# t-taniai/LocalExpStereo

Measured on AMD Instinct MI355X. Metric: Mcost-evals/s (pixels x hypotheses / s), guided-filter cost aggregation, 1500x1000x256 vol, higher is better.
Workload: dtype i32 fixed-point box sums (exact; i64 stage-2 window sums), f32 3x3 algebra and combination

## Files before the change

localexpstereo_amd/csrc/les_hip.hip:

```cpp
#include "../../include/localexp_hip.h"
#include "les_kernels.h"
#include "les_march.h"
#include "les_propose.h"
#include "les_post.h"
#include "les_pairwise.h"
#include "les_maxflow.h"
#include "les_maxflow_tiled.h"
#include "les_maxflow_cell.h"

#include "../host/ResidualCut.h"

#include <algorithm>
#include <atomic>
#include <chrono>
#include <cstdint>
#include <mutex>
#if !defined(LES_SIM)
#include <dlfcn.h>
#endif
#include <cstdarg>
#include <cstdio>
#include <cstdlib>
#include <cstring>
#include <string>
#include <vector>

namespace {

thread_local std::string g_err;

int fail(int code, const char* fmt, ...)
{
    char buf[512];
    va_list ap;
    va_start(ap, fmt);
    vsnprintf(buf, sizeof buf, fmt, ap);
    va_end(ap);
    g_err = buf;
    return code;
}

enum FallbackReason { FB_RADIUS = 0, FB_NONFINITE, FB_RANGE, FB_THRESHOLD, FB_IMAGE_SIZE, FB_GEOMETRY, FB_PATCHES, FB_GUIDE, FB_COUNT };
void note_fallback(std::atomic<unsigned>& seen, FallbackReason r, const char* fmt, ...)
{
    if (seen.fetch_or(1u << r, std::memory_order_relaxed) & (1u << r)) return;
    static const bool quiet = [] { const char* e = getenv("LES_HIP_QUIET"); return e && atoi(e) != 0; }();
    if (quiet) return;
    char buf[512];
    va_list ap;
    va_start(ap, fmt);
    vsnprintf(buf, sizeof buf, fmt, ap);
    va_end(ap);
    fprintf(stderr, "localexp_hip: strip kernel instead of the march kernel: %s (LES_HIP_QUIET=1 silences this note)\n", buf);
}

#define HIPCHECK(expr)                                                                               \
    do {                                                                                             \
        hipError_t e_ = (expr);                                                                      \
        if (e_ != hipSuccess)                                                                        \
            return fail(LES_HIP_ERR_DEVICE, "%s failed: %s (%s:%d)", #expr, hipGetErrorString(e_), __FILE__, __LINE__); \
    } while (0)

#include "les_hip_march_tables.inc"

struct ViewData {
    float* vol = nullptr;
    bool own_vol = false;
    float4* stats = nullptr;
    uint32_t* ipk = nullptr;
    uint32_t* ipk10 = nullptr;
    float4* feat = nullptr;
    uint32_t* ipk8 = nullptr;
    float* mstats = nullptr;
    float* vol_t = nullptr;
    bool march_ok = false;
    unsigned dmax_bits = 0;
    les::MarchView mv = {};
};

}

struct MtHost;
namespace { void mt_host_free(MtHost* m); }

struct les_hip_ctx {
    les_hip_params p;
    int R;
    const StripEntry* strip;
    const MarchEntry* march = nullptr;
    int ncu = 256;
    std::atomic<unsigned> fallback_seen{0};
    hipStream_t stream;
    les::Geom geom;
    ViewData v[2];
    float naive_alpha = 0;
    int naive = 0;
    float th_color = 0, th_grad = 0;
    float4* d_planes = nullptr; size_t planes_cap = 0;
    float* d_map = nullptr;
    les::WtaJob* d_wta = nullptr; size_t wta_cap = 0;
    float4* d_wta_planes = nullptr; size_t wta_planes_cap = 0;
    float* d_pw_tab = nullptr; float pw_omega = -1.f, pw_epsilon = -1.f;
    std::mutex mu;
    unsigned long long gen = 0;
    std::vector<les_hip_scratch*> idle_scratch;
    bool maxflow_lds_ready = false;
    bool maxflow_tiled_lds_ready = false;
    std::vector<les_hip_scratch*> own_scratch;
    std::vector<MtHost*> mt_idle;
};

struct les_hip_batch {
    int n = 0, njobs = 0, out_slabs = 0, R = 0;
    les::Job* d_jobs = nullptr;
    les::Job* d_mjobs = nullptr;
    const MarchEntry* mentry = nullptr;
    int nmgroups = 0;
    bool march_ok = false;
    les::RawCall* d_rawcalls = nullptr;
    long long* d_raw_off = nullptr;
    long long raw_floats = 0;
    int raw_chunks = 1;
    mutable float* d_raw[2] = {nullptr, nullptr};
    std::vector<les_hip_rect> targets;
    int device = 0;
    les::Rect4* d_units = nullptr;
    les::WtaJob* d_targets = nullptr;
    les::RansacScratch rs = {nullptr, nullptr, nullptr, nullptr, nullptr, nullptr, 0, nullptr};
    int wta_chunks = 1;
    int graph_chunks = 1;
    std::vector<long long> graph_off;
    long long graph_nodes = 0;
    long long* d_graph_off = nullptr;
    double* d_flow0 = nullptr;
    mutable std::mutex mt_mu;
    mutable les::MtTile* d_mt_tiles = nullptr;
    mutable int* d_mt_tiles_per_cell = nullptr;
    mutable int mt_ntiles = -1;
    mutable std::mutex mf_mu;
    mutable int* d_mf_list = nullptr;
    mutable int mf_list_key = -1;
    mutable int mf_count[3] = {0, 0, 0};
};

struct les_hip_scratch {
    les_hip_ctx* c = nullptr;
    hipStream_t stream = nullptr;
    float* d_tile = nullptr; float* h_tile = nullptr; size_t tile_cap = 0;
    float4* d_plane = nullptr; float4* h_plane = nullptr;
    struct Entry { les_hip_rect f, t; int want_march; const void* march; int njobs, ngroups; les::Job* d_jobs; unsigned long long stamp; };
    float* d_raw = nullptr; size_t raw_cap = 0;
    les::RawCall* d_rawcall = nullptr; long long* d_raw_off = nullptr;
    les_hip_rect raw_f = {-1, -1, -1, -1};
    std::vector<Entry> cache;
    unsigned long long clock = 0;
};

namespace {

std::atomic<unsigned long long> g_ctx_gen{0};
std::mutex g_live_mu;
std::vector<std::pair<unsigned long long, les_hip_ctx*>> g_live;
void release_hidden_scratch(unsigned long long gen, les_hip_scratch* s)
{
    std::lock_guard<std::mutex> lk(g_live_mu);
    for (auto& e : g_live)
        if (e.first == gen) {
            std::lock_guard<std::mutex> lk2(e.second->mu);
            e.second->idle_scratch.push_back(s);
            return;
        }
}
thread_local unsigned long long tl_stream_gen = 0;
thread_local hipStream_t tl_stream = nullptr;
inline hipStream_t cur_stream(const les_hip_ctx* c) { return (tl_stream_gen != 0 && tl_stream_gen == c->gen) ? tl_stream : c->stream; }

#include "les_hip_march.inc"

float naive_alpha(const les_hip_ctx* c) { return c->naive_alpha; }

}

#include "les_hip_context.inc"
#include "les_hip_batch.inc"
#include "les_hip_cuts.inc"
#include "les_hip_ingest_post.inc"
#include "les_hip_exchange.inc"
```

localexpstereo_amd/csrc/les_hip_batch.inc:

```
extern "C" {

int les_hip_batch_create(les_hip_ctx* c, int n, const les_hip_rect* frs, const les_hip_rect* trs, int out_slabs, les_hip_batch** out)
{
    if (!c || !out || n < 0 || (n > 0 && (!frs || !trs))) return fail(LES_HIP_ERR_ARG, "null argument");
    if (out_slabs < 0) return fail(LES_HIP_ERR_ARG, "out_slabs must be 0 (one map) or the number of consecutive calls that share a slab");
    if (out_slabs > 1 && n % out_slabs != 0) return fail(LES_HIP_ERR_ARG, "out_slabs = %d does not divide the %d calls of the batch (slab i / out_slabs holds out_slabs consecutive calls; pass 1 for one slab per call)", out_slabs, n);
    *out = nullptr;
    std::vector<les::Job> jobs;
    int rc = build_jobs(c, n, frs, trs, out_slabs, jobs);
    if (rc) return rc;
    les_hip_batch* b = new les_hip_batch();
    b->n = n; b->njobs = (int)jobs.size(); b->out_slabs = out_slabs; b->R = c->R; b->device = c->p.device;
    b->targets.assign(trs, trs + n);
    {
        int max_area = 1;
        for (int i = 0; i < n; i++) max_area = std::max(max_area, trs[i].w * trs[i].h);
        b->wta_chunks = std::min(32, std::max(1, (max_area + 4095) / 4096));
        b->graph_chunks = std::min(256, std::max(1, (max_area + 255) / 256));
    }
    b->graph_off.resize((size_t)n);
    for (int i = 0; i < n; i++) {
        b->graph_off[i] = b->graph_nodes;
        b->graph_nodes += (long long)std::max(0, trs[i].w) * std::max(0, trs[i].h);
    }
    if (n > 0) {
        static_assert(sizeof(les::WtaJob) == sizeof(les_hip_rect), "rect layout");
        static_assert(sizeof(les::GraphCell) == sizeof(les_hip_rect), "rect layout");
        if (hipMalloc((void**)&b->d_graph_off, (size_t)n * sizeof(long long)) != hipSuccess ||
            hipMemcpy(b->d_graph_off, b->graph_off.data(), (size_t)n * sizeof(long long), hipMemcpyHostToDevice) != hipSuccess ||
            hipMalloc((void**)&b->d_flow0, (size_t)n * b->graph_chunks * sizeof(double)) != hipSuccess) {
            les_hip_batch_destroy(b);
            return fail(LES_HIP_ERR_DEVICE, "upload of the graph offset table failed");
        }
        if (hipMalloc((void**)&b->d_targets, (size_t)n * sizeof(les::WtaJob)) != hipSuccess ||
            hipMemcpy(b->d_targets, trs, (size_t)n * sizeof(les::WtaJob), hipMemcpyHostToDevice) != hipSuccess) {
            les_hip_batch_destroy(b);
            return fail(LES_HIP_ERR_DEVICE, "upload of the target table failed");
        }
    }
    {
        std::vector<les::Job> mjobs;
        bool mok = false;
        build_march_jobs(c, n, frs, trs, out_slabs, mjobs, mok, b->mentry);
        if (mok && !mjobs.empty()) {
            if (hipMalloc((void**)&b->d_mjobs, mjobs.size() * sizeof(les::Job)) != hipSuccess ||
                hipMemcpy(b->d_mjobs, mjobs.data(), mjobs.size() * sizeof(les::Job), hipMemcpyHostToDevice) != hipSuccess) {
                les_hip_batch_destroy(b);
                return fail(LES_HIP_ERR_DEVICE, "upload of the march job table failed");
            }
            b->nmgroups = (int)(mjobs.size() / b->mentry->NJ);
            b->march_ok = true;
        }
        if (b->march_ok && c->naive) {
            std::vector<les::RawCall> calls((size_t)n);
            std::vector<long long> offs((size_t)n);
            long long tot = 0, amax = 1;
            for (int i = 0; i < n; i++) {
                const bool live = trs[i].w > 0 && trs[i].h > 0;
                const long long a = live ? (long long)frs[i].w * frs[i].h : 0;
                calls[i] = les::RawCall{frs[i].x, frs[i].y, live ? frs[i].w : 0, live ? frs[i].h : 0, tot};
                offs[i] = tot;
                tot += a; amax = std::max(amax, a);
            }
            if (tot > kRawPatchCapFloats) {
                b->march_ok = false;
                note_fallback(c->fallback_seen, FB_PATCHES, "the raw-cost patches of one batch of the image-based energy exceed 4 GB");
            }
            else {
                b->raw_floats = tot;
                b->raw_chunks = (int)std::min<long long>(1024, std::max<long long>(1, (amax + 4095) / 4096));
                if (hipMalloc((void**)&b->d_rawcalls, (size_t)n * sizeof(les::RawCall)) != hipSuccess ||
                    hipMemcpy(b->d_rawcalls, calls.data(), (size_t)n * sizeof(les::RawCall), hipMemcpyHostToDevice) != hipSuccess ||
                    hipMalloc((void**)&b->d_raw_off, (size_t)n * sizeof(long long)) != hipSuccess ||
                    hipMemcpy(b->d_raw_off, offs.data(), (size_t)n * sizeof(long long), hipMemcpyHostToDevice) != hipSuccess) {
                    les_hip_batch_destroy(b);
                    return fail(LES_HIP_ERR_DEVICE, "upload of the raw-cost call table failed");
                }
            }
        }
    }
    if (!jobs.empty()) {
        if (hipMalloc((void**)&b->d_jobs, jobs.size() * sizeof(les::Job)) != hipSuccess) { les_hip_batch_destroy(b); return fail(LES_HIP_ERR_DEVICE, "hipMalloc(jobs) failed"); }
        if (hipMemcpy(b->d_jobs, jobs.data(), jobs.size() * sizeof(les::Job), hipMemcpyHostToDevice) != hipSuccess) {
            les_hip_batch_destroy(b); return fail(LES_HIP_ERR_DEVICE, "hipMemcpy(jobs) failed");
        }
    }
    *out = b;
    return LES_HIP_OK;
}

void les_hip_batch_destroy(les_hip_batch* b)
{
    if (!b) return;
    if (b->d_jobs) (void)hipFree(b->d_jobs);
    if (b->d_mjobs) (void)hipFree(b->d_mjobs);
    if (b->d_rawcalls) (void)hipFree(b->d_rawcalls);
    if (b->d_raw_off) (void)hipFree(b->d_raw_off);
    for (int m = 0; m < 2; m++) if (b->d_raw[m]) (void)hipFree(b->d_raw[m]);
    if (b->d_units) (void)hipFree(b->d_units);
    if (b->d_targets) (void)hipFree(b->d_targets);
    if (b->d_graph_off) (void)hipFree(b->d_graph_off);
    if (b->d_flow0) (void)hipFree(b->d_flow0);
    if (b->d_mt_tiles) (void)hipFree(b->d_mt_tiles);
    if (b->d_mt_tiles_per_cell) (void)hipFree(b->d_mt_tiles_per_cell);
    if (b->d_mf_list) (void)hipFree(b->d_mf_list);
    if (b->rs.disp) (void)hipFree(b->rs.disp);
    if (b->rs.idx) (void)hipFree(b->rs.idx);
    if (b->rs.state) (void)hipFree(b->rs.state);
    if (b->rs.noi) (void)hipFree(b->rs.noi);
    if (b->rs.no) (void)hipFree(b->rs.no);
    if (b->rs.refit) (void)hipFree(b->rs.refit);
    if (b->rs.cell) (void)hipFree(b->rs.cell);
    delete b;
}

int les_hip_batch_set_units(les_hip_ctx* c, les_hip_batch* b, const les_hip_rect* units)
{
    if (!c || !b || (b->n > 0 && !units)) return fail(LES_HIP_ERR_ARG, "null argument");
    int maxlen = 1;
    for (int i = 0; i < b->n; i++) {
        const les_hip_rect& u = units[i];
        if (u.w <= 0 || u.h <= 0 || u.x < 0 || u.y < 0 || u.x + u.w > c->p.W || u.y + u.h > c->p.H)
            return fail(LES_HIP_ERR_ARG, "unit rect %d empty or outside the image", i);
        maxlen = std::max(maxlen, u.w * u.h);
    }
    if (b->n == 0) return LES_HIP_OK;
    static_assert(sizeof(les::Rect4) == sizeof(les_hip_rect), "rect layout");
    if (!b->d_units) HIPCHECK(hipMalloc((void**)&b->d_units, (size_t)b->n * sizeof(les::Rect4)));
    HIPCHECK(hipMemcpy(b->d_units, units, (size_t)b->n * sizeof(les::Rect4), hipMemcpyHostToDevice));
    if (!b->rs.idx) {
        const size_t n = (size_t)b->n, S = kRansacMaxSam;
        HIPCHECK(hipMalloc((void**)&b->rs.idx, n * S * 3 * sizeof(int)));
        HIPCHECK(hipMalloc((void**)&b->rs.state, n * (S + 1) * sizeof(uint64_t)));
        HIPCHECK(hipMalloc((void**)&b->rs.noi, n * S * sizeof(int)));
        HIPCHECK(hipMalloc((void**)&b->rs.no, n * S * sizeof(int)));
        HIPCHECK(hipMalloc((void**)&b->rs.refit, n * S * 3 * sizeof(float)));
        HIPCHECK(hipMalloc((void**)&b->rs.cell, n * sizeof(les::RansacCell)));
    }
    if (b->rs.disp) HIPCHECK(hipFree(b->rs.disp));
    b->rs.disp = nullptr;
    b->rs.stride = maxlen;
    HIPCHECK(hipMalloc((void**)&b->rs.disp, (size_t)b->n * maxlen * sizeof(float)));
    return LES_HIP_OK;
}

int les_hip_batch_propose(les_hip_ctx* c, const les_hip_batch* b, int kind, int m, les_hip_plane* labels, uint64_t* rng,
                          les_hip_plane* planes)
{
    if (c) (void)hipSetDevice(c->p.device);
    if (!c || !b || !labels || !rng || !planes) return fail(LES_HIP_ERR_ARG, "null argument");
    if (b->n == 0) return LES_HIP_OK;
    if (!b->d_units) return fail(LES_HIP_ERR_ARG, "les_hip_batch_set_units was not called for this batch");
    float4* lab = reinterpret_cast<float4*>(labels);
    float4* pl = reinterpret_cast<float4*>(planes);
    const int n = b->n, W = c->p.W;
    const float mind = c->p.min_disparity, maxd = c->p.max_disparity;
    switch (kind) {
    case LES_HIP_PROPOSE_EXPANSION:
        hipLaunchKernelGGL(les::les_expansion_kernel, dim3((n + 63) / 64), dim3(64), 0, cur_stream(c), b->d_units, lab, W, rng, pl, n);
        break;
    case LES_HIP_PROPOSE_RANDOM:
        hipLaunchKernelGGL(les::les_random_kernel, dim3((n + 63) / 64), dim3(64), 0, cur_stream(c), b->d_units, lab, W, rng, pl, n, m, mind, maxd);
        break;
    case LES_HIP_PROPOSE_RANSAC:
        hipLaunchKernelGGL(les::les_ransac_snapshot_kernel, dim3(n), dim3(256), 0, cur_stream(c), b->d_units, lab, W, b->rs);
        hipLaunchKernelGGL(les::les_ransac_begin_kernel, dim3((n + 63) / 64), dim3(64), 0, cur_stream(c), b->d_units, rng, b->rs, n, kRansacMaxSam, kRansacChunkEnds[0]);
        for (int k = 0, j0 = 0; k < kRansacChunks; k++) {
            const int j1 = kRansacChunkEnds[k], j2 = k + 1 < kRansacChunks ? kRansacChunkEnds[k + 1] : kRansacMaxSam;
            hipLaunchKernelGGL(les::les_ransac_eval_kernel, dim3(n, (j1 - j0 + les::kRansacCandPerBlock - 1) / les::kRansacCandPerBlock), dim3(64 * les::kRansacCandPerBlock), 0, cur_stream(c), b->d_units, b->rs, kRansacMaxSam, 1.0f, j0, j1);
            hipLaunchKernelGGL(les::les_ransac_walk_kernel, dim3((n + 63) / 64), dim3(64), 0, cur_stream(c), b->d_units, rng, pl, b->rs, n, kRansacMaxSam, 0.95f, j0, j1, j2);
            j0 = j1;
        }
        break;
    case LES_HIP_PROPOSE_INIT:
        hipLaunchKernelGGL(les::les_init_labels_kernel, dim3(n), dim3(64), 0, cur_stream(c), b->d_units, lab, W, rng, pl, mind, maxd);
        break;
    default:
        return fail(LES_HIP_ERR_ARG, "unknown proposer kind %d", kind);
    }
    HIPCHECK(hipGetLastError());
    return LES_HIP_OK;
}

int les_hip_batch_wta(les_hip_ctx* c, const les_hip_batch* b, const les_hip_plane* planes, float* cur, const float* prop,
                      les_hip_plane* labels)
{
    if (c) (void)hipSetDevice(c->p.device);
    if (!c || !b || !planes || !cur || !prop || !labels) return fail(LES_HIP_ERR_ARG, "null argument");
    if (b->n == 0) return LES_HIP_OK;
    if (!b->d_targets) return fail(LES_HIP_ERR_ARG, "batch has no target table");
    hipLaunchKernelGGL(les::les_wta_kernel, dim3(b->n, b->wta_chunks), dim3(256), 0, cur_stream(c), b->d_targets, reinterpret_cast<const float4*>(planes),
                       cur, prop, reinterpret_cast<float4*>(labels), c->p.W);
    HIPCHECK(hipGetLastError());
    return LES_HIP_OK;
}

int les_hip_batch_num_jobs(const les_hip_batch* b) { return b ? (b->march_ok ? b->nmgroups : b->njobs) : 0; }

int les_hip_batch_kernel_kind(const les_hip_ctx* c, const les_hip_batch* b, int mode)
{
    if (!c || !b || mode < 0 || mode > 1) return -1;
    return (b->march_ok && c->march && c->v[mode].march_ok) ? 1 : 0;
}

int les_hip_batch_run(les_hip_ctx* c, const les_hip_batch* b, int mode, const les_hip_plane* planes, int planes_on_device,
                      float* out_dev, int check)
{
    if (c) (void)hipSetDevice(c->p.device);
    if (!c || !b || !out_dev || (b->n > 0 && !planes)) return fail(LES_HIP_ERR_ARG, "null argument");
    if (b->R != c->R) return fail(LES_HIP_ERR_ARG, "batch was prepared for a different context");
    const float4* d_planes = reinterpret_cast<const float4*>(planes);
    if (!planes_on_device) {
        int rc = ensure_planes(c, (size_t)b->n);
        if (rc) return rc;
        HIPCHECK(hipMemcpyAsync(c->d_planes, planes, (size_t)b->n * sizeof(float4), hipMemcpyHostToDevice, cur_stream(c)));
        d_planes = c->d_planes;
    }
    if (b->march_ok && mode >= 0 && mode <= 1 && c->march && c->v[mode].march_ok) {
        if (!c->naive) return launch_march(c, b->mentry, mode, b->d_mjobs, b->nmgroups, d_planes, out_dev, check, cur_stream(c));
        {
            std::lock_guard<std::mutex> lk(c->mu);
            if (!b->d_raw[mode]) HIPCHECK(hipMalloc((void**)&b->d_raw[mode], (size_t)std::max<long long>(b->raw_floats, 1) * sizeof(float)));
        }
        const RawPatches rp{b->d_rawcalls, b->d_raw_off, b->d_raw[mode], b->n, b->raw_chunks};
        return launch_march(c, b->mentry, mode, b->d_mjobs, b->nmgroups, d_planes, out_dev, check, cur_stream(c), &rp);
    }
    return launch_strips(c, mode, b->d_jobs, b->njobs, d_planes, out_dev, check, cur_stream(c));
}

int les_hip_unary_batch(les_hip_ctx* c, int mode, int n, const les_hip_rect* frs, const les_hip_rect* trs,
                        const les_hip_plane* planes, float* cost_map, int check)
{
    if (!c || !cost_map) return fail(LES_HIP_ERR_ARG, "null argument");
    les_hip_batch* b = nullptr;
    int rc = les_hip_batch_create(c, n, frs, trs, 0, &b);
    if (rc) return rc;
    rc = les_hip_batch_run(c, b, mode, planes, 0, c->d_map, check);
    if (rc == LES_HIP_OK) {
        for (int i = 0; i < n && rc == LES_HIP_OK; i++) {
            const les_hip_rect& t = trs[i];
            if (t.w <= 0 || t.h <= 0) continue;
            size_t off = (size_t)t.y * c->p.W + t.x;
            hipError_t e = hipMemcpy2DAsync(cost_map + off, (size_t)c->p.W * sizeof(float), c->d_map + off, (size_t)c->p.W * sizeof(float),
                                            (size_t)t.w * sizeof(float), (size_t)t.h, hipMemcpyDeviceToHost, cur_stream(c));
            if (e != hipSuccess) rc = fail(LES_HIP_ERR_DEVICE, "hipMemcpy2DAsync failed: %s", hipGetErrorString(e));
        }
        if (rc == LES_HIP_OK && hipStreamSynchronize(cur_stream(c)) != hipSuccess) rc = fail(LES_HIP_ERR_DEVICE, "stream synchronize failed");
    }
    les_hip_batch_destroy(b);
    return rc;
}

int les_hip_scratch_create(les_hip_ctx* c, les_hip_scratch** out)
{
    if (!c || !out) return fail(LES_HIP_ERR_ARG, "null argument");
    *out = nullptr;
    HIPCHECK(hipSetDevice(c->p.device));
    les_hip_scratch* s = new les_hip_scratch();
    s->c = c;
    if (hipStreamCreateWithFlags(&s->stream, hipStreamNonBlocking) != hipSuccess ||
        hipMalloc((void**)&s->d_plane, sizeof(float4)) != hipSuccess || hipHostMalloc((void**)&s->h_plane, sizeof(float4), hipHostMallocDefault) != hipSuccess) {
        les_hip_scratch_destroy(s);
        return fail(LES_HIP_ERR_DEVICE, "scratch allocation failed");
    }
    *out = s;
    return LES_HIP_OK;
}

void les_hip_scratch_destroy(les_hip_scratch* s)
{
    if (!s) return;
    if (s->c) (void)hipSetDevice(s->c->p.device);
    if (s->stream) { (void)hipStreamSynchronize(s->stream); (void)hipStreamDestroy(s->stream); }
    for (auto& e : s->cache) if (e.d_jobs) (void)hipFree(e.d_jobs);
    if (s->d_tile) (void)hipFree(s->d_tile);
    if (s->h_tile) (void)hipHostFree(s->h_tile);
    if (s->d_raw) (void)hipFree(s->d_raw);
    if (s->d_rawcall) (void)hipFree(s->d_rawcall);
    if (s->d_raw_off) (void)hipFree(s->d_raw_off);
    if (s->d_plane) (void)hipFree(s->d_plane);
    if (s->h_plane) (void)hipHostFree(s->h_plane);
    delete s;
}

int les_hip_unary_one_scratch(les_hip_ctx* c, les_hip_scratch* s, int mode, const les_hip_rect* fr, const les_hip_rect* tr,
                              const les_hip_plane* plane, float* costs, int row_stride, int check)
{
    if (!c || !s || !fr || !tr || !plane || !costs) return fail(LES_HIP_ERR_ARG, "null argument");
    if (s->c != c) return fail(LES_HIP_ERR_ARG, "scratch belongs to another context");
    if (mode < 0 || mode > 1 || !c->v[mode].stats || (c->naive ? !c->v[1 - mode].feat : !c->v[mode].vol))
        return fail(LES_HIP_ERR_ARG, "view %d was not supplied at creation", mode);
    HIPCHECK(hipSetDevice(c->p.device));
    int rc = check_rects(c, *fr, *tr);
    if (rc) return rc;
    if (tr->w <= 0 || tr->h <= 0) return LES_HIP_OK;
    const int want_march = (c->march && c->v[mode].march_ok) ? 1 : 0;
    les_hip_scratch::Entry* e = nullptr;
    for (auto& x : s->cache)
        if (x.want_march == want_march && !memcmp(&x.f, fr, sizeof *fr) && !memcmp(&x.t, tr, sizeof *tr)) { e = &x; break; }
    if (!e) {
        std::vector<les::Job> jobs;
        bool mok = false;
        const MarchEntry* me = nullptr;
        if (want_march) build_march_jobs(c, 1, fr, tr, 0, jobs, mok, me);
        const bool use_march = want_march && mok && !jobs.empty();
        if (!use_march) {
            rc = build_jobs(c, 1, fr, tr, 0, jobs);
            if (rc) return rc;
            me = nullptr;
        }
        for (auto& j : jobs) {
            j.out_off = (long long)(j.ty0 - tr->y) * tr->w + (j.tx0 - tr->x);
            j.out_stride = tr->w;
        }
        les_hip_scratch::Entry ne{*fr, *tr, want_march, me, (int)jobs.size(), me ? (int)(jobs.size() / me->NJ) : 0, nullptr, 0};
        if (s->cache.size() >= 16) {
            size_t k = 0;
            for (size_t i = 1; i < s->cache.size(); i++) if (s->cache[i].stamp < s->cache[k].stamp) k = i;
            HIPCHECK(hipStreamSynchronize(s->stream));
            if (s->cache[k].d_jobs) HIPCHECK(hipFree(s->cache[k].d_jobs));
            s->cache.erase(s->cache.begin() + (long)k);
        }
        HIPCHECK(hipMalloc((void**)&ne.d_jobs, jobs.size() * sizeof(les::Job)));
        if (hipMemcpy(ne.d_jobs, jobs.data(), jobs.size() * sizeof(les::Job), hipMemcpyHostToDevice) != hipSuccess) {
            (void)hipFree(ne.d_jobs);
            return fail(LES_HIP_ERR_DEVICE, "upload of the job table failed");
        }
        s->cache.push_back(ne);
        e = &s->cache.back();
    }
    e->stamp = ++s->clock;
    const size_t need = (size_t)tr->w * tr->h;
    if (need > s->tile_cap) {
        HIPCHECK(hipStreamSynchronize(s->stream));
        if (s->d_tile) HIPCHECK(hipFree(s->d_tile));
        if (s->h_tile) HIPCHECK(hipHostFree(s->h_tile));
        s->d_tile = nullptr; s->h_tile = nullptr; s->tile_cap = 0;
        const size_t cap = std::max(need, (size_t)256 * 256);
        HIPCHECK(hipMalloc((void**)&s->d_tile, cap * sizeof(float)));
        HIPCHECK(hipHostMalloc((void**)&s->h_tile, cap * sizeof(float), hipHostMallocDefault));
        s->tile_cap = cap;
    }
    *s->h_plane = make_float4(plane->a, plane->b, plane->c, plane->v);
    HIPCHECK(hipMemcpyAsync(s->d_plane, s->h_plane, sizeof(float4), hipMemcpyHostToDevice, s->stream));
    if (e->march && c->naive) {
        const size_t rneed = (size_t)fr->w * fr->h;
        if (rneed > s->raw_cap || !s->d_rawcall) {
            HIPCHECK(hipStreamSynchronize(s->stream));
            if (s->d_raw) HIPCHECK(hipFree(s->d_raw));
            s->d_raw = nullptr; s->raw_cap = 0;
            const size_t cap = std::max(rneed, (size_t)256 * 256);
            HIPCHECK(hipMalloc((void**)&s->d_raw, cap * sizeof(float)));
            s->raw_cap = cap;
            if (!s->d_rawcall) {
                HIPCHECK(hipMalloc((void**)&s->d_rawcall, sizeof(les::RawCall)));
                HIPCHECK(hipMalloc((void**)&s->d_raw_off, sizeof(long long)));
                const long long zero = 0;
                HIPCHECK(hipMemcpy(s->d_raw_off, &zero, sizeof zero, hipMemcpyHostToDevice));
            }
            s->raw_f = les_hip_rect{-1, -1, -1, -1};
        }
        if (memcmp(&s->raw_f, fr, sizeof *fr)) {
            const les::RawCall call{fr->x, fr->y, fr->w, fr->h, 0};
            HIPCHECK(hipStreamSynchronize(s->stream));
            HIPCHECK(hipMemcpy(s->d_rawcall, &call, sizeof call, hipMemcpyHostToDevice));
            s->raw_f = *fr;
        }
        const RawPatches rp{s->d_rawcall, s->d_raw_off, s->d_raw, 1, (int)std::min<size_t>(1024, (rneed + 4095) / 4096)};
        rc = launch_march(c, static_cast<const MarchEntry*>(e->march), mode, e->d_jobs, e->ngroups, s->d_plane, s->d_tile, check, s->stream, &rp);
    }
    else if (e->march) rc = launch_march(c, static_cast<const MarchEntry*>(e->march), mode, e->d_jobs, e->ngroups, s->d_plane, s->d_tile, check, s->stream);
    else rc = launch_strips(c, mode, e->d_jobs, e->njobs, s->d_plane, s->d_tile, check, s->stream);
    if (rc) return rc;
    HIPCHECK(hipMemcpyAsync(s->h_tile, s->d_tile, need * sizeof(float), hipMemcpyDeviceToHost, s->stream));
    HIPCHECK(hipStreamSynchronize(s->stream));
    float* dst = costs + (size_t)(tr->y - fr->y) * row_stride + (tr->x - fr->x);
    for (int y = 0; y < tr->h; y++) memcpy(dst + (size_t)y * row_stride, s->h_tile + (size_t)y * tr->w, (size_t)tr->w * sizeof(float));
    return LES_HIP_OK;
}

int les_hip_unary_one(les_hip_ctx* c, int mode, const les_hip_rect* fr, const les_hip_rect* tr, const les_hip_plane* plane,
                      float* costs, int row_stride, int check)
{
    if (!c || !fr || !tr || !plane || !costs) return fail(LES_HIP_ERR_ARG, "null argument");
    struct Mine {
        std::vector<std::pair<unsigned long long, les_hip_scratch*>> v;
        ~Mine() { for (auto& e : v) release_hidden_scratch(e.first, e.second); }
    };
    thread_local Mine mine;
    les_hip_scratch* s = nullptr;
    for (auto& e : mine.v) if (e.first == c->gen) { s = e.second; break; }
    if (!s) {
        {
            std::lock_guard<std::mutex> lk(c->mu);
            if (!c->idle_scratch.empty()) { s = c->idle_scratch.back(); c->idle_scratch.pop_back(); }
        }
        if (!s) {
            int rc = les_hip_scratch_create(c, &s);
            if (rc) return rc;
            std::lock_guard<std::mutex> lk(c->mu);
            c->own_scratch.push_back(s);
        }
        mine.v.emplace_back(c->gen, s);
    }
    return les_hip_unary_one_scratch(c, s, mode, fr, tr, plane, costs, row_stride, check);
}

int les_hip_wta_update(les_hip_ctx* c, int n, const les_hip_rect* rects, const les_hip_plane* planes, int planes_on_device,
                       float* cur, const float* prop, les_hip_plane* labels)
{
    if (!c || n < 0 || (n > 0 && (!rects || !planes || !cur || !prop || !labels))) return fail(LES_HIP_ERR_ARG, "null argument");
    if (n == 0) return LES_HIP_OK;
    for (int i = 0; i < n; i++)
        if (rects[i].x < 0 || rects[i].y < 0 || rects[i].w < 0 || rects[i].h < 0 || rects[i].x + rects[i].w > c->p.W || rects[i].y + rects[i].h > c->p.H)
            return fail(LES_HIP_ERR_ARG, "rect outside the image");
    if ((size_t)n > c->wta_cap) {
        if (c->d_wta) HIPCHECK(hipFree(c->d_wta));
        c->d_wta = nullptr; c->wta_cap = 0;
        HIPCHECK(hipMalloc((void**)&c->d_wta, std::max<size_t>(n, 1024) * sizeof(les::WtaJob)));
        c->wta_cap = std::max<size_t>(n, 1024);
    }
    static_assert(sizeof(les::WtaJob) == sizeof(les_hip_rect), "rect layout");
    HIPCHECK(hipMemcpyAsync(c->d_wta, rects, (size_t)n * sizeof(les::WtaJob), hipMemcpyHostToDevice, cur_stream(c)));
    const float4* d_planes = reinterpret_cast<const float4*>(planes);
    if (!planes_on_device) {
        if ((size_t)n > c->wta_planes_cap) {
            if (c->d_wta_planes) HIPCHECK(hipFree(c->d_wta_planes));
            c->d_wta_planes = nullptr; c->wta_planes_cap = 0;
            HIPCHECK(hipMalloc((void**)&c->d_wta_planes, std::max<size_t>(n, 1024) * sizeof(float4)));
            c->wta_planes_cap = std::max<size_t>(n, 1024);
        }
        HIPCHECK(hipMemcpyAsync(c->d_wta_planes, planes, (size_t)n * sizeof(float4), hipMemcpyHostToDevice, cur_stream(c)));
        d_planes = c->d_wta_planes;
    }
    int max_area = 1;
    for (int i = 0; i < n; i++) max_area = std::max(max_area, rects[i].w * rects[i].h);
    const int chunks = std::min(32, std::max(1, (max_area + 4095) / 4096));
    hipLaunchKernelGGL(les::les_wta_kernel, dim3(n, chunks), dim3(256), 0, cur_stream(c), c->d_wta, d_planes, cur, prop,
                       reinterpret_cast<float4*>(labels), c->p.W);
    HIPCHECK(hipGetLastError());
    return LES_HIP_OK;
}

}
```

localexpstereo_amd/csrc/les_hip_context.inc:

```
extern "C" {

const char* les_hip_last_error(void) { return g_err.c_str(); }

#if defined(LES_PHASE_TIMING)
int les_hip_debug_phases(unsigned long long* out)
{
    (void)hipDeviceSynchronize();
    if (hipMemcpyFromSymbol(out, HIP_SYMBOL(les::les_dbg), 12 * sizeof(unsigned long long)) != hipSuccess) return 1;
    unsigned long long z[12] = {0, 0, 0, 0, 0, 0, 0, 0, 0, 0, 0, 0};
    (void)hipMemcpyToSymbol(HIP_SYMBOL(les::les_dbg), z, sizeof z);
    return 0;
}
#endif

int les_hip_strip_width(int R)
{
    const StripEntry* e = find_strip(R);
    return e ? e->TW : 0;
}

static int create_common(les_hip_ctx** out, const les_hip_params* params, const uint8_t* imL, const uint8_t* imR,
                         const float* volL, const float* volR, int naive, float alpha, float th_grad)
{
    if (!out || !params) return fail(LES_HIP_ERR_ARG, "null argument");
    *out = nullptr;
    les_hip_params p = *params;
    if (naive) { p.D = 1; p.volumes_on_device = 0; }
    if (p.H <= 0 || p.W <= 0 || p.D <= 0 || p.windR < 2) return fail(LES_HIP_ERR_ARG, "bad dimensions");
    if (naive && (!imL || !imR)) return fail(LES_HIP_ERR_ARG, "the image-based matching cost needs both views");
    if ((unsigned long long)p.H * p.W * p.D >= (1ull << 32)) return fail(LES_HIP_ERR_UNSUPPORTED, "volumes of 2^32 or more floats are not supported (32-bit element offsets)");
    const StripEntry* strip = naive ? find_naive_strip(p.windR / 2) : find_strip(p.windR / 2);
    if (!strip) return fail(LES_HIP_ERR_UNSUPPORTED, "no kernel instantiated for guided-filter radius %d (windR %d)", p.windR / 2, p.windR);
    int ndev = 0;
    if (hipGetDeviceCount(&ndev) != hipSuccess || ndev <= 0) return fail(LES_HIP_ERR_DEVICE, "no HIP device available (this library has no CPU fallback)");
    if (p.device < 0 || p.device >= ndev) return fail(LES_HIP_ERR_ARG, "device %d out of range (%d devices)", p.device, ndev);
    HIPCHECK(hipSetDevice(p.device));
    les_hip_ctx* c = new les_hip_ctx();
    c->gen = ++g_ctx_gen;
    { std::lock_guard<std::mutex> lk(g_live_mu); g_live.emplace_back(c->gen, c); }
    c->p = p;
    c->R = p.windR / 2;
    c->strip = strip;
    c->march = find_march(p.windR / 2);
    if (!c->march && !(getenv("LES_HIP_KERNEL") && !strcmp(getenv("LES_HIP_KERNEL"), "strip")))
        note_fallback(c->fallback_seen, FB_RADIUS, "no march kernel for guided-filter radius %d (windR %d; instantiated: 2 .. 10)", p.windR / 2, p.windR);
#if !defined(LES_SIM)
    {
        int v = 0;
        if (hipDeviceGetAttribute(&v, hipDeviceAttributeMultiprocessorCount, p.device) == hipSuccess && v > 0) c->ncu = v;
    }
#endif
    c->stream = nullptr;
    c->geom.H = p.H; c->geom.W = p.W; c->geom.D = p.D;
    c->geom.D0 = (int)(-p.min_disparity);
    c->geom.th_col = p.th_col; c->geom.pad_ = 0.0f;
    c->geom.maxd = p.max_disparity; c->geom.mind = p.min_disparity;
    c->naive = naive;
    if (naive) {
        c->th_color = p.th_col * (1.0f - alpha);
        c->th_grad = th_grad * alpha;
        c->naive_alpha = alpha;
    }
    const uint8_t* ims[2] = {imL, imR};
    const float* vols[2] = {volL, volR};
    for (int m = 0; m < 2; m++) {
        int rc = build_view(c, m, ims[m], vols[m]);
        if (rc) { les_hip_destroy(c); return rc; }
    }
    if (hipMalloc((void**)&c->d_map, (size_t)p.H * p.W * sizeof(float)) != hipSuccess) {
        les_hip_destroy(c);
        return fail(LES_HIP_ERR_DEVICE, "hipMalloc of the scratch cost map failed");
    }
    *out = c;
    return LES_HIP_OK;
}

int les_hip_create(les_hip_ctx** out, const les_hip_params* params, const uint8_t* imL, const uint8_t* imR,
                   const float* volL, const float* volR)
{
    return create_common(out, params, imL, imR, volL, volR, 0, 0.0f, 0.0f);
}

int les_hip_create_naive(les_hip_ctx** out, const les_hip_params* params, const uint8_t* imL, const uint8_t* imR, float alpha, float th_grad)
{
    return create_common(out, params, imL, imR, nullptr, nullptr, 1, alpha, th_grad);
}

void les_hip_destroy(les_hip_ctx* c)
{
    if (!c) return;
    (void)hipSetDevice(c->p.device);
    if (tl_stream_gen == c->gen) { tl_stream_gen = 0; tl_stream = nullptr; }
    {
        std::lock_guard<std::mutex> lk(g_live_mu);
        g_live.erase(std::remove_if(g_live.begin(), g_live.end(), [c](const std::pair<unsigned long long, les_hip_ctx*>& e) { return e.second == c; }), g_live.end());
    }
    for (int m = 0; m < 2; m++) {
        if (c->v[m].own_vol && c->v[m].vol) (void)hipFree(c->v[m].vol);
        if (c->v[m].stats) (void)hipFree(c->v[m].stats);
        if (c->v[m].ipk) (void)hipFree(c->v[m].ipk);
        if (c->v[m].ipk10) (void)hipFree(c->v[m].ipk10);
        if (c->v[m].feat) (void)hipFree(c->v[m].feat);
        if (c->v[m].ipk8) (void)hipFree(c->v[m].ipk8);
        if (c->v[m].mstats) (void)hipFree(c->v[m].mstats);
        if (c->v[m].vol_t) (void)hipFree(c->v[m].vol_t);
    }
    for (les_hip_scratch* sc : c->own_scratch) les_hip_scratch_destroy(sc);
    c->own_scratch.clear();
    for (MtHost* m : c->mt_idle) mt_host_free(m);
    c->mt_idle.clear();
    if (c->d_planes) (void)hipFree(c->d_planes);
    if (c->d_map) (void)hipFree(c->d_map);
    if (c->d_wta) (void)hipFree(c->d_wta);
    if (c->d_wta_planes) (void)hipFree(c->d_wta_planes);
    if (c->d_pw_tab) (void)hipFree(c->d_pw_tab);
    delete c;
}

int les_hip_set_stream(les_hip_ctx* c, void* s)
{
    if (!c) return fail(LES_HIP_ERR_ARG, "null context");
    c->stream = (hipStream_t)s;
    return LES_HIP_OK;
}

int les_hip_set_thread_stream(les_hip_ctx* c, void* s, int bind)
{
    if (!c) return fail(LES_HIP_ERR_ARG, "null context");
    if (bind) { tl_stream_gen = c->gen; tl_stream = (hipStream_t)s; }
    else if (tl_stream_gen == c->gen) { tl_stream_gen = 0; tl_stream = nullptr; }
    return LES_HIP_OK;
}

int les_hip_synchronize(les_hip_ctx* c)
{
    if (!c) return fail(LES_HIP_ERR_ARG, "null context");
    HIPCHECK(hipStreamSynchronize(cur_stream(c)));
    return LES_HIP_OK;
}

int les_hip_refresh_volume(les_hip_ctx* c, int mode)
{
    if (!c) return fail(LES_HIP_ERR_ARG, "null argument");
    if (mode < 0 || mode > 1 || !c->v[mode].vol) return fail(LES_HIP_ERR_ARG, "view %d has no cost volume", mode);
    HIPCHECK(hipSetDevice(c->p.device));
    std::lock_guard<std::mutex> lk(c->mu);
    HIPCHECK(hipStreamSynchronize(cur_stream(c)));
    if (!c->march || !c->v[mode].mstats) return LES_HIP_OK;
    const int rc = build_march_view(c, mode, nullptr);
    if (rc) return rc;
    HIPCHECK(hipStreamSynchronize(cur_stream(c)));
    return LES_HIP_OK;
}

int les_hip_calib_copy(const float* d_src, float* d_dst, size_t n, int device, void* stream)
{
    if (!d_src || !d_dst || n == 0) return fail(LES_HIP_ERR_ARG, "bad argument");
    HIPCHECK(hipSetDevice(device));
    hipLaunchKernelGGL(les::les_calib_copy_kernel, dim3((unsigned)((n + 255) / 256)), dim3(256), 0, (hipStream_t)stream, d_src, d_dst, n);
    HIPCHECK(hipGetLastError());
    return LES_HIP_OK;
}

int les_hip_calib_copy_wide(const float* d_src, float* d_dst, size_t n, int device, void* stream)
{
    if (!d_src || !d_dst || n == 0 || (n & 3) || (((uintptr_t)d_src | (uintptr_t)d_dst) & 15)) return fail(LES_HIP_ERR_ARG, "bad argument (n must be a multiple of 4, pointers 16-byte aligned)");
    HIPCHECK(hipSetDevice(device));
    const size_t n4 = n / 4;
    hipLaunchKernelGGL(les::les_calib_copy_wide_kernel, dim3((unsigned)((n4 + 1023) / 1024)), dim3(256), 0, (hipStream_t)stream,
                       reinterpret_cast<const float4*>(d_src), reinterpret_cast<float4*>(d_dst), n4);
    HIPCHECK(hipGetLastError());
    return LES_HIP_OK;
}

int les_hip_malloc(les_hip_ctx* c, void** p, size_t bytes)
{
    if (!c || !p) return fail(LES_HIP_ERR_ARG, "null argument");
    HIPCHECK(hipMalloc(p, bytes));
    return LES_HIP_OK;
}
int les_hip_free(les_hip_ctx* c, void* p)
{
    if (!c) return fail(LES_HIP_ERR_ARG, "null argument");
    if (p) HIPCHECK(hipFree(p));
    return LES_HIP_OK;
}
int les_hip_memcpy_h2d(les_hip_ctx* c, void* d, const void* s, size_t bytes)
{
    if (!c) return fail(LES_HIP_ERR_ARG, "null argument");
    HIPCHECK(hipMemcpyAsync(d, s, bytes, hipMemcpyHostToDevice, cur_stream(c)));
    HIPCHECK(hipStreamSynchronize(cur_stream(c)));
    return LES_HIP_OK;
}
int les_hip_memcpy_d2h(les_hip_ctx* c, void* d, const void* s, size_t bytes)
{
    if (!c) return fail(LES_HIP_ERR_ARG, "null argument");
    HIPCHECK(hipMemcpyAsync(d, s, bytes, hipMemcpyDeviceToHost, cur_stream(c)));
    HIPCHECK(hipStreamSynchronize(cur_stream(c)));
    return LES_HIP_OK;
}
int les_hip_memset(les_hip_ctx* c, void* d, int value, size_t bytes)
{
    if (!c) return fail(LES_HIP_ERR_ARG, "null argument");
    HIPCHECK(hipMemsetAsync(d, value, bytes, cur_stream(c)));
    return LES_HIP_OK;
}

size_t les_hip_tiled_volume_bytes(les_hip_ctx* c, int mode)
{
    if (!c || mode < 0 || mode > 1 || !c->v[mode].vol_t) return 0;
    return (size_t)c->p.H * (size_t)((c->p.W + 7) / 8) * 8u * (size_t)c->p.D * sizeof(float);
}

int les_hip_get_stats(les_hip_ctx* c, int mode, float* out)
{
    if (!c || !out || mode < 0 || mode > 1 || !c->v[mode].stats) return fail(LES_HIP_ERR_ARG, "bad argument");
    HIPCHECK(hipMemcpy(out, c->v[mode].stats, (size_t)c->p.H * c->p.W * 12 * sizeof(float), hipMemcpyDeviceToHost));
    return LES_HIP_OK;
}

}
```

localexpstereo_amd/csrc/les_hip_march.inc:

```
int check_rects(const les_hip_ctx* c, const les_hip_rect& f, const les_hip_rect& t)
{
    if (f.w < 0 || f.h < 0 || t.w < 0 || t.h < 0) return fail(LES_HIP_ERR_ARG, "negative rect size");
    if (f.x < 0 || f.y < 0 || f.x + f.w > c->p.W || f.y + f.h > c->p.H) return fail(LES_HIP_ERR_ARG, "filterRect outside the image");
    if (t.w > 0 && t.h > 0 && (t.x < f.x || t.y < f.y || t.x + t.w > f.x + f.w || t.y + t.h > f.y + f.h))
        return fail(LES_HIP_ERR_ARG, "targetRect not inside filterRect");
    return LES_HIP_OK;
}

int build_jobs(const les_hip_ctx* c, int n, const les_hip_rect* frs, const les_hip_rect* trs, int out_slabs,
               std::vector<les::Job>& jobs)
{
    const int TW = c->strip->TW, R = c->R;
    const long long P = (long long)c->p.H * c->p.W;
    long long strips = 0;
    for (int i = 0; i < n; i++) {
        int rc = check_rects(c, frs[i], trs[i]);
        if (rc) return rc;
        if (trs[i].w > 0 && trs[i].h > 0) strips += (trs[i].w + TW - 1) / TW;
    }
    int max_rows = 1 << 30;
    if (strips > 0 && strips < 2048) {
        long long want = (2048 + strips - 1) / strips;
        int tallest = 0;
        for (int i = 0; i < n; i++) tallest = std::max(tallest, trs[i].h);
        max_rows = std::max<long long>(std::max(8 * R, 64), (tallest + want - 1) / want);
    }
    jobs.clear();
    for (int i = 0; i < n; i++) {
        const les_hip_rect &f = frs[i], &t = trs[i];
        if (t.w <= 0 || t.h <= 0) continue;
        for (int sy = 0; sy < t.h; sy += max_rows)
            for (int sx = 0; sx < t.w; sx += TW) {
                les::Job j;
                j.tx0 = t.x + sx; j.ty0 = t.y + sy;
                j.tw = std::min(TW, t.w - sx); j.th = std::min(max_rows, t.h - sy);
                j.cx0 = f.x; j.cy0 = f.y; j.cx1 = f.x + f.w; j.cy1 = f.y + f.h;
                j.out_off = (out_slabs ? (long long)(i / out_slabs) * P : 0) + (long long)j.ty0 * c->p.W + j.tx0;
                j.out_stride = c->p.W;
                j.plane_idx = i;
                jobs.push_back(j);
            }
    }
    std::stable_sort(jobs.begin(), jobs.end(), [](const les::Job& a, const les::Job& b) {
        if (a.tx0 != b.tx0) return a.tx0 < b.tx0;
        if (a.ty0 != b.ty0) return a.ty0 < b.ty0;
        return a.plane_idx < b.plane_idx;
    });
    return LES_HIP_OK;
}

bool build_march_jobs(les_hip_ctx* c, int n, const les_hip_rect* frs, const les_hip_rect* trs, int out_slabs,
                      std::vector<les::Job>& jobs, bool& ok, const MarchEntry*& entry)
{
    jobs.clear();
    ok = false;
    entry = nullptr;
    if (!c->march) return true;
    const int R = c->R, W = c->p.W, H = c->p.H;
    const long long P = (long long)H * W;
    ok = true;
    for (int i = 0; i < n; i++) {
        const les_hip_rect &f = frs[i], &t = trs[i];
        if (t.w <= 0 || t.h <= 0) continue;
        if ((f.x > 0 && t.x - f.x < 2 * R) || (f.x + f.w < W && (f.x + f.w) - (t.x + t.w) < 2 * R) ||
            (f.y > 0 && t.y - f.y < 2 * R) || (f.y + f.h < H && (f.y + f.h) - (t.y + t.h) < 2 * R)) ok = false;
    }
    if (!ok) {
        note_fallback(c->fallback_seen, FB_GEOMETRY, "a target rectangle lies closer than 2 x radius = %d pixels to a filterRect border that is not an image border", 2 * R);
        return true;
    }
    const int ncu = c->ncu;
    const MarchEntry* cands[2] = {c->march, find_march(c->R, 0)};
    const MarchEntry* m = c->march;
    int max_rows = 1 << 30;
    {
        double best = 1e300;
        const int row_opts[] = {1 << 30, 1024, 512, 384, 256, 192, 128, 96, 64, 48, 32};
        for (int g = 0; g < 2; g++) {
            const MarchEntry* e = cands[g];
            if (!e || (g == 1 && e == cands[0])) continue;
            if (const char* w = getenv("LES_HIP_MARCH_WIDE")) if ((atoi(w) != 0) != (g == 0)) continue;
            for (int ro : row_opts) {
                long long njobs = 0;
                int rows = 0, useful = 0;
                for (int i = 0; i < n; i++) {
                    const les_hip_rect& t = trs[i];
                    if (t.w <= 0 || t.h <= 0) continue;
                    const int ns = (t.w + e->TW - 1) / e->TW;
                    const int nr = (t.h + ro - 1) / ro, sh = (t.h + nr - 1) / nr;
                    njobs += (long long)ns * nr;
                    rows = std::max(rows, sh);
                    useful = std::max(useful, (t.w + ns - 1) / ns);
                }
                if (njobs == 0) continue;
                const long long wgs = (njobs + e->NJ - 1) / e->NJ;
                const double ticks = (double)((rows + 4 * R + e->BY - 1) / e->BY + 3);
                const double cost = (double)((wgs + ncu - 1) / ncu) * ticks * (1.0 + 1e-3 * (double)wgs / ncu) + (ro == (1 << 30) ? 0.0 : 1e-6);
                if (cost < best) { best = cost; m = e; max_rows = ro; }
            }
        }
    }
    if (const char* e = getenv("LES_HIP_MARCH_ROWS")) max_rows = std::max(1, atoi(e));
    entry = m;
    const int TW = m->TW, NJ = m->NJ;
    for (int i = 0; i < n; i++) {
        const les_hip_rect &f = frs[i], &t = trs[i];
        if (t.w <= 0 || t.h <= 0) continue;
        const int ns = (t.w + TW - 1) / TW, sw = (t.w + ns - 1) / ns;
        const int nr = (t.h + max_rows - 1) / max_rows, sh = (t.h + nr - 1) / nr;
        for (int sy = 0; sy < t.h; sy += sh)
            for (int sx = 0; sx < t.w; sx += sw) {
                les::Job j;
                j.tx0 = t.x + sx; j.ty0 = t.y + sy;
                j.tw = std::min(sw, t.w - sx); j.th = std::min(sh, t.h - sy);
                j.cx0 = f.x; j.cy0 = f.y; j.cx1 = f.x + f.w; j.cy1 = f.y + f.h;
                j.out_off = (out_slabs ? (long long)(i / out_slabs) * P : 0) + (long long)j.ty0 * W + j.tx0;
                j.out_stride = W;
                j.plane_idx = i;
                jobs.push_back(j);
            }
    }
    std::stable_sort(jobs.begin(), jobs.end(), [](const les::Job& a, const les::Job& b) {
        if (a.tx0 != b.tx0) return a.tx0 < b.tx0;
        if (a.ty0 != b.ty0) return a.ty0 < b.ty0;
        return a.plane_idx < b.plane_idx;
    });
    while (!jobs.empty() && jobs.size() % NJ) {
        les::Job pad = jobs.back();
        pad.tw = 0; pad.th = 0;
        jobs.push_back(pad);
    }
    return true;
}

int ensure_planes(les_hip_ctx* c, size_t n)
{
    if (n <= c->planes_cap) return LES_HIP_OK;
    if (c->d_planes) HIPCHECK(hipFree(c->d_planes));
    c->d_planes = nullptr; c->planes_cap = 0;
    size_t cap = std::max<size_t>(n, 1024);
    HIPCHECK(hipMalloc((void**)&c->d_planes, cap * sizeof(float4)));
    c->planes_cap = cap;
    return LES_HIP_OK;
}

struct RawPatches { const les::RawCall* calls; const long long* off; float* raw; int n, chunks; };

les::View strip_view(const les_hip_ctx* c, int mode)
{
    les::View view{c->v[mode].vol, c->v[mode].stats, c->v[mode].ipk, c->v[mode].ipk10, nullptr, nullptr, mode ? -1.0f : 1.0f, c->th_color, c->th_grad};
    if (c->naive) { view.feat_self = c->v[mode].feat; view.feat_other = c->v[1 - mode].feat; }
    return view;
}

int launch_march(les_hip_ctx* c, const MarchEntry* m, int mode, const les::Job* d_mjobs, int ngroups, const float4* d_planes, float* d_out, int check,
                 hipStream_t stream, const RawPatches* rp = nullptr)
{
    if (ngroups <= 0) return LES_HIP_OK;
    les::MarchView mv = c->v[mode].mv;
    if (c->naive) {
        if (!rp || !rp->raw || !c->v[1 - mode].feat) return fail(LES_HIP_ERR_ARG, "view %d was not supplied at creation", mode);
        hipLaunchKernelGGL(les::les_naive_raw_kernel, dim3(rp->n, rp->chunks), dim3(256), 0, stream, c->geom, strip_view(c, mode), rp->calls, d_planes, rp->raw);
        mv.vol = rp->raw; mv.raw_off = rp->off;
    }
    hipLaunchKernelGGL(m->fn, dim3(ngroups), dim3(m->NT), 0, stream, c->geom, mv, d_mjobs, d_planes, d_out, ngroups, check);
    HIPCHECK(hipGetLastError());
    return LES_HIP_OK;
}

int launch_strips(les_hip_ctx* c, int mode, const les::Job* d_jobs, int njobs, const float4* d_planes, float* d_out, int check, hipStream_t stream)
{
    if (njobs <= 0) return LES_HIP_OK;
    if (mode < 0 || mode > 1 || !c->v[mode].stats || (c->naive ? !c->v[1 - mode].feat : !c->v[mode].vol))
        return fail(LES_HIP_ERR_ARG, "view %d was not supplied at creation", mode);
    const les::View view = strip_view(c, mode);
    hipLaunchKernelGGL(c->strip->fn, dim3(njobs), dim3(c->strip->NT), 0, stream, c->geom, view, d_jobs, d_planes, d_out, njobs, check);
    HIPCHECK(hipGetLastError());
    return LES_HIP_OK;
}

float naive_alpha(const les_hip_ctx* c);

int build_march_view(les_hip_ctx* c, int m, const double* d_hs)
{
    ViewData& v = c->v[m];
    const size_t P = (size_t)c->p.H * c->p.W;
    const int W = c->p.W, H = c->p.H;
    v.march_ok = false;
    if ((unsigned long long)P * (4ull * les::kMarchStatWords) >= (1ull << 31)) {
        note_fallback(c->fallback_seen, FB_IMAGE_SIZE, "image of %d x %d pixels (32-bit row offsets reach 2^26 pixels)", W, H);
        return LES_HIP_OK;
    }
    const float th = c->naive ? c->th_color + c->th_grad : c->p.th_col;
    if (!(th > 0.0f) || !(th < INFINITY)) { note_fallback(c->fallback_seen, FB_THRESHOLD, "truncation threshold %g is not positive and finite", (double)th); return LES_HIP_OK; }
    if (d_hs) {
        unsigned dbits = 0;
        struct DevBuf { void* p = nullptr; ~DevBuf() { if (p) (void)hipFree(p); } } dm;
        HIPCHECK(hipMalloc(&dm.p, sizeof(unsigned)));
        unsigned* d_dmax = static_cast<unsigned*>(dm.p);
        HIPCHECK(hipMemsetAsync(d_dmax, 0, sizeof(unsigned), cur_stream(c)));
        HIPCHECK(hipMalloc((void**)&v.ipk8, P * sizeof(uint32_t)));
        HIPCHECK(hipMalloc((void**)&v.mstats, P * les::kMarchStatWords * sizeof(float)));
        hipLaunchKernelGGL(les::les_march_stats_kernel, dim3((W + 255) / 256, H), dim3(256), 0, cur_stream(c), d_hs, v.ipk, v.ipk8, v.mstats, d_dmax, H, W, c->R, c->p.eps);
        HIPCHECK(hipGetLastError());
        HIPCHECK(hipMemcpyAsync(&dbits, d_dmax, sizeof(unsigned), hipMemcpyDeviceToHost, cur_stream(c)));
        HIPCHECK(hipStreamSynchronize(cur_stream(c)));
        v.dmax_bits = dbits;
    }
    auto drop_tiled = [&]() { if (v.vol_t) { (void)hipFree(v.vol_t); v.vol_t = nullptr; } };
    const int nb = 2048;
    std::vector<float> hmin(nb, 0.0f); std::vector<int> hbad(nb, 0);
    if (!c->naive) {
        struct DevBuf { void* p = nullptr; ~DevBuf() { if (p) (void)hipFree(p); } } part;
        HIPCHECK(hipMalloc(&part.p, nb * (sizeof(float) + sizeof(int))));
        float* d_min = static_cast<float*>(part.p);
        int* d_bad = reinterpret_cast<int*>(d_min + nb);
        hipLaunchKernelGGL(les::les_range_kernel, dim3(nb), dim3(256), 0, cur_stream(c), v.vol, P * (size_t)c->p.D, d_min, d_bad);
        HIPCHECK(hipGetLastError());
        HIPCHECK(hipMemcpyAsync(hmin.data(), d_min, nb * sizeof(float), hipMemcpyDeviceToHost, cur_stream(c)));
        HIPCHECK(hipMemcpyAsync(hbad.data(), d_bad, nb * sizeof(int), hipMemcpyDeviceToHost, cur_stream(c)));
        HIPCHECK(hipStreamSynchronize(cur_stream(c)));
    }
    float vmin = INFINITY; int bad = 0;
    for (int i = 0; i < nb; i++) { vmin = std::min(vmin, hmin[i]); bad |= hbad[i]; }
    if (bad || !(vmin < INFINITY)) {
        note_fallback(c->fallback_seen, FB_NONFINITE, "the cost volume of view %d holds NaN or infinite entries", m);
        drop_tiled();
        return LES_HIP_OK;
    }
    vmin = std::min(vmin, 0.5f * th);
    const double range = (double)th - (double)vmin;
    if (!(range <= 8.0 * (double)th)) {
        note_fallback(c->fallback_seen, FB_RANGE, "view %d: costs reach %g below the truncation threshold %g (more than 8 x the threshold)", m, range, (double)th);
        drop_tiled();
        return LES_HIP_OK;
    }
    const unsigned dbits = v.dmax_bits;
    float dmax;
    memcpy(&dmax, &dbits, sizeof dmax);
    if (!(dmax > 0.0f) || !(dmax < INFINITY)) { note_fallback(c->fallback_seen, FB_GUIDE, "view %d: the inverse covariance of the guide is not positive and finite (largest diagonal entry %g)", m, (double)dmax); return LES_HIP_OK; }
    const int K = 2 * c->R + 1;
    const double Ba = 0.5 * range * std::sqrt((double)dmax), Bb = range + 1.5 * Ba;
    const double scale = 1073741824.0 / ((double)K * Bb * 1.25);
    const int PB = les::march_pb(c->R);
    const float spf = (float)((double)((1 << PB) - 1) / range);
    const double c0 = std::rint(-(double)vmin * (double)spf) - (double)(1 << (PB - 1));
    const double up = 1.0 / (double)spf;
    les::MarchView mv;
    mv.vol = v.vol; mv.ipk8 = v.ipk8; mv.mstats = v.mstats;
    mv.sp = spf;
    mv.pmagic = (float)(12582912.0 + c0);
    mv.poff = (float)(-c0 * up);
    mv.kapS = (float)((double)(1 << les::kMarchSH) * up / 255.0 * scale);
    mv.upS = (float)(up * scale);
    mv.qscale = (float)((double)(1 << les::kMarchS2) / (255.0 * scale));
    mv.kmu = (float)(1.0 / ((double)(1ll << les::kMarchMB) * 255.0));
    mv.raw_off = nullptr;
    mv.vol_t = nullptr;
    if (!c->naive && v.vol) {
        const char* e = getenv("LES_HIP_TILED");
        const unsigned long long nt = (unsigned long long)H * (unsigned long long)((W + 7) / 8) * 8ull * (unsigned long long)c->p.D;
        if (!(e && atoi(e) == 0) && (unsigned long long)((W + 7) / 8) * (unsigned long long)c->p.D * 32ull < (1ull << 31)) {
            if (v.vol_t) { (void)hipFree(v.vol_t); v.vol_t = nullptr; }
            size_t mem_free = 0, mem_total = 0;
            const bool room = hipMemGetInfo(&mem_free, &mem_total) == hipSuccess && mem_free >= 2 * nt * sizeof(float) + (4ull << 30);
            if (room && hipMalloc((void**)&v.vol_t, nt * sizeof(float)) == hipSuccess) {
                hipLaunchKernelGGL(les::les_tile_volume_kernel, dim3((unsigned)(((W + 7) / 8 * 8 + 63) / 64), (unsigned)H), dim3(256), 0, cur_stream(c), v.vol, v.vol_t, c->p.D, H, W);
                HIPCHECK(hipGetLastError());
                mv.vol_t = v.vol_t;
            } else {
                (void)hipGetLastError();
                v.vol_t = nullptr;
            }
        }
    }
    v.mv = mv;
    v.march_ok = true;
    return LES_HIP_OK;
}

int build_view(les_hip_ctx* c, int m, const uint8_t* im, const float* vol)
{
    const size_t P = (size_t)c->p.H * c->p.W;
    ViewData& v = c->v[m];
    if (vol) {
        if (c->p.volumes_on_device) { v.vol = const_cast<float*>(vol); v.own_vol = false; }
        else {
            HIPCHECK(hipMalloc((void**)&v.vol, P * c->p.D * sizeof(float)));
            v.own_vol = true;
            HIPCHECK(hipMemcpy(v.vol, vol, P * c->p.D * sizeof(float), hipMemcpyHostToDevice));
        }
    }
    if (!im) return LES_HIP_OK;
    uint8_t* d_img = nullptr;
    double* d_hs = nullptr;
    HIPCHECK(hipMalloc((void**)&d_img, P * 3));
    HIPCHECK(hipMemcpy(d_img, im, P * 3, hipMemcpyHostToDevice));
    HIPCHECK(hipMalloc((void**)&v.ipk, P * sizeof(uint32_t)));
    HIPCHECK(hipMalloc((void**)&v.ipk10, P * sizeof(uint32_t)));
    HIPCHECK(hipMalloc((void**)&v.stats, (P * 3 + 1) * sizeof(float4)));
    HIPCHECK(hipMemsetAsync(v.stats + P * 3, 0, sizeof(float4), cur_stream(c)));
    HIPCHECK(hipMalloc((void**)&d_hs, P * 9 * sizeof(double)));
    const int W = c->p.W, H = c->p.H;
    if (c->naive) {
        HIPCHECK(hipMalloc((void**)&v.feat, P * sizeof(float4)));
        hipLaunchKernelGGL(les::les_naive_features_kernel, dim3((c->p.W + 255) / 256, c->p.H), dim3(256), 0, cur_stream(c), d_img, v.feat, c->p.H, c->p.W, naive_alpha(c));
    }
    hipLaunchKernelGGL(les::les_pack_guide_kernel, dim3((unsigned)((P + 255) / 256)), dim3(256), 0, cur_stream(c), d_img, v.ipk, v.ipk10, (int)P);
    hipLaunchKernelGGL(les::les_stats_hsum_kernel, dim3((W + 255) / 256, H), dim3(256), 0, cur_stream(c), v.ipk, d_hs, H, W, c->R);
    hipLaunchKernelGGL(les::les_stats_finish_kernel, dim3((W + 255) / 256, H), dim3(256), 0, cur_stream(c), d_hs, v.stats, H, W, c->R, c->p.eps);
    HIPCHECK(hipGetLastError());
    if (c->march && (v.vol || c->naive)) {
        int rc = build_march_view(c, m, d_hs);
        if (rc) { (void)hipFree(d_img); (void)hipFree(d_hs); return rc; }
    }
    HIPCHECK(hipStreamSynchronize(cur_stream(c)));
    HIPCHECK(hipFree(d_img));
    HIPCHECK(hipFree(d_hs));
    return LES_HIP_OK;
}
```

localexpstereo_amd/csrc/les_hip_march_tables.inc:

```
typedef void (*StripKernel)(les::Geom, les::View, const les::Job*, const float4*, float*, int, int);
struct StripEntry { int R; int variant; int TW; int NT; StripKernel fn; };

#define LES_STRIP_ENTRY(R_, V_, WA_, BY_, SEG_, MW_) \
    { R_, V_, les::StripCfg<R_, WA_, BY_, SEG_>::TW, les::StripCfg<R_, WA_, BY_, SEG_>::NT, les::les_strip_kernel<R_, WA_, BY_, SEG_, MW_> }
const StripEntry kStrips[] = {
    LES_STRIP_ENTRY(1, 0, 64, 16, 4, 2), LES_STRIP_ENTRY(2, 0, 64, 16, 4, 2), LES_STRIP_ENTRY(3, 0, 64, 16, 4, 2),
    LES_STRIP_ENTRY(4, 0, 64, 16, 4, 2), LES_STRIP_ENTRY(5, 0, 64, 16, 4, 2), LES_STRIP_ENTRY(6, 0, 64, 16, 4, 2),
    LES_STRIP_ENTRY(7, 0, 64, 16, 4, 2), LES_STRIP_ENTRY(8, 0, 64, 16, 4, 2), LES_STRIP_ENTRY(9, 0, 64, 16, 4, 2),
    LES_STRIP_ENTRY(10, 0, 64, 21, 3, 3), LES_STRIP_ENTRY(12, 0, 64, 16, 4, 2), LES_STRIP_ENTRY(15, 0, 96, 16, 6, 2),
    LES_STRIP_ENTRY(10, 8, 128, 21, 6, 2), LES_STRIP_ENTRY(10, 11, 64, 21, 3, 2),
};
#define LES_NAIVE_ENTRY(R_, WA_, BY_, SEG_, MW_) \
    { R_, 0, les::StripCfg<R_, WA_, BY_, SEG_>::TW, les::StripCfg<R_, WA_, BY_, SEG_>::NT, les::les_strip_kernel<R_, WA_, BY_, SEG_, MW_, 1> }
const StripEntry kNaiveStrips[] = {
    LES_NAIVE_ENTRY(1, 64, 16, 4, 2), LES_NAIVE_ENTRY(2, 64, 16, 4, 2), LES_NAIVE_ENTRY(3, 64, 16, 4, 2), LES_NAIVE_ENTRY(4, 64, 16, 4, 2),
    LES_NAIVE_ENTRY(5, 64, 16, 4, 2), LES_NAIVE_ENTRY(6, 64, 16, 4, 2), LES_NAIVE_ENTRY(7, 64, 16, 4, 2), LES_NAIVE_ENTRY(8, 64, 16, 4, 2),
    LES_NAIVE_ENTRY(9, 64, 16, 4, 2), LES_NAIVE_ENTRY(10, 64, 16, 4, 2), LES_NAIVE_ENTRY(12, 64, 16, 4, 2), LES_NAIVE_ENTRY(15, 96, 16, 6, 2),
};
const StripEntry* find_naive_strip(int R)
{
    for (const auto& e : kNaiveStrips)
        if (e.R == R) return &e;
    return nullptr;
}
const StripEntry* find_strip(int R)
{
    int variant = 0;
    if (const char* v = getenv("LES_HIP_VARIANT")) variant = atoi(v);
    const StripEntry* def = nullptr;
    for (const auto& e : kStrips) {
        if (e.R != R) continue;
        if (e.variant == variant) return &e;
        if (e.variant == 0) def = &e;
    }
    return def;
}

typedef void (*MarchKernel)(les::Geom, les::MarchView, const les::Job*, const float4*, float*, int, int);
struct MarchEntry { int R; int TW; int NJ; int NT; int BY; MarchKernel fn; };
#define LES_MARCH_ENTRY(R_, WGC_, NJ_, BY_) \
    { R_, les::MarchCfg<R_, WGC_, NJ_, BY_>::TW, NJ_, les::MarchCfg<R_, WGC_, NJ_, BY_>::NT, BY_, les::les_march_kernel<R_, WGC_, NJ_, BY_> }
const MarchEntry kMarch[] = {
    LES_MARCH_ENTRY(10, 256, 1, 7),
#if defined(LES_MARCH_LAB) && defined(LES_MARCH_NARROW_NJ1)
    LES_MARCH_ENTRY(10, 128, 1, 7),
#else
    LES_MARCH_ENTRY(10, 128, 2, 7),
#endif
    LES_MARCH_ENTRY(7, 256, 1, 5),
    LES_MARCH_ENTRY(7, 128, 2, 5),
#if !defined(LES_MARCH_FEW_RADII)
    LES_MARCH_ENTRY(2, 256, 1, 2),  LES_MARCH_ENTRY(2, 128, 2, 2),
    LES_MARCH_ENTRY(3, 256, 1, 3),  LES_MARCH_ENTRY(3, 128, 2, 3),
    LES_MARCH_ENTRY(4, 256, 1, 3),  LES_MARCH_ENTRY(4, 128, 2, 3),
    LES_MARCH_ENTRY(5, 256, 1, 4),  LES_MARCH_ENTRY(5, 128, 2, 4),
    LES_MARCH_ENTRY(6, 256, 1, 5),  LES_MARCH_ENTRY(6, 128, 2, 5),
    LES_MARCH_ENTRY(8, 256, 1, 6),  LES_MARCH_ENTRY(8, 128, 2, 6),
    LES_MARCH_ENTRY(9, 256, 1, 7),  LES_MARCH_ENTRY(9, 128, 2, 7),
#endif
};
const MarchEntry* find_march(int R, int wide = 1)
{
    if (const char* k = getenv("LES_HIP_KERNEL")) if (!strcmp(k, "strip")) return nullptr;
    const MarchEntry* best = nullptr;
    for (const auto& e : kMarch)
        if (e.R == R && (!best || (wide ? e.TW > best->TW : e.TW < best->TW))) best = &e;
    return best;
}

constexpr long long kRawPatchCapFloats = 1ll << 30;
constexpr int kRansacMaxSam = 500;
constexpr int kRansacChunks = 5;
constexpr int kRansacChunkEnds[kRansacChunks] = {16, 64, 128, 256, kRansacMaxSam};
```

localexpstereo_amd/csrc/les_kernels.h:

```cpp
#pragma once

#include "les_simt.h"

#include <utility>

namespace les {

struct Geom {
    int H, W, D, D0;
    float th_col, pad_;
    float maxd, mind;
};

struct View {
    const float* vol;
    const float4* stats;
    const uint32_t* ipk;
    const uint32_t* ipk10;
    const float4* feat_self;
    const float4* feat_other;
    float sign;
    float th_color, th_grad;
};

struct Job {
    int tx0, ty0, tw, th;
    int cx0, cy0, cx1, cy1;
    long long out_off;
    int out_stride;
    int plane_idx;
};

#define LES_COST_INVALID 1000000.0f

__device__ __forceinline__ float gather_cost(const Geom& g, const float* __restrict__ vol, float a, float b,
                                             float c, int gx, int gy)
{
    const size_t HW = (size_t)g.H * g.W;
    const size_t px = (size_t)gy * g.W + gx;
    float d_base = b * (float)gy + c;
    float d = a * (float)gx + d_base;
    float C;
    if (d < g.mind) C = vol[px];
    else if (d >= g.maxd) C = vol[(size_t)(g.D - 1) * HW + px];
    else if (d != d || fabsf(d) == INFINITY) C = LES_COST_INVALID;
    else {
        int d0 = (int)d + g.D0;
        int d1 = d0 + 1;
        float f1 = d - floorf(d);
        float f0 = 1.0f - f1;
        if (d1 >= g.D || d0 < 0) C = LES_COST_INVALID;
        else {
            float v0 = vol[(size_t)d0 * HW + px];
            float v1 = vol[(size_t)d1 * HW + px];
            C = f0 * v0 + f1 * v1;
        }
    }
    return (g.th_col < C) ? g.th_col : C;
}

struct GatherPrep {
    uint32_t i0, i1;
    float f1;
    int mode;
};
__device__ __forceinline__ GatherPrep gather_prepare(const Geom& g, float ax, float d_base, uint32_t px, uint32_t HW, bool inside)
{
    GatherPrep r;
    const float d = ax + d_base;
    const bool lo = d < g.mind, hi = d >= g.maxd;
    const bool mid = !(lo || hi || d != d);
    const float dsafe = mid ? d : 0.0f;
    const int d0 = (int)dsafe + g.D0;
    const bool ok = mid && d0 >= 0 && d0 + 1 < g.D;
    r.f1 = dsafe - floorf(dsafe);
    const uint32_t s0 = lo ? 0u : (hi ? (uint32_t)(g.D - 1) : (ok ? (uint32_t)d0 : 0u));
    r.i0 = s0 * HW + px;
    r.i1 = ok ? r.i0 + HW : r.i0;
    r.mode = !inside ? 3 : ((lo || hi) ? 1 : (ok ? 0 : 2));
    return r;
}
__device__ __forceinline__ float gather_finish(const Geom& g, const GatherPrep& r, float v0, float v1)
{
    const float f0 = 1.0f - r.f1;
    float C = f0 * v0 + r.f1 * v1;
    C = r.mode == 1 ? v0 : C;
    C = r.mode == 2 ? LES_COST_INVALID : C;
    const float p = (g.th_col < C) ? g.th_col : C;
    return r.mode == 3 ? 0.0f : p;
}

struct NaivePrep {
    uint32_t ia, ib;
    float w1;
};
__device__ __forceinline__ NaivePrep naive_prepare(const Geom& g, float sign, float a, float b, float c, int gx, int gy)
{
    NaivePrep r;
    const float z = (a * (float)gx + b * (float)gy) + c;
    const double sx = (double)gx - (double)sign * (double)z;
    const double q = floor(sx * 32.0 + 0.5) / 32.0;
    const double fl = floor(q);
    r.w1 = (float)(q - fl);
    const double flc = fmin(fmax(fl, -2.0), (double)g.W + 1.0);
    const int x0 = (int)flc;
    const int xa = min(max(x0, 0), g.W - 1), xb = min(max(x0 + 1, 0), g.W - 1);
    r.ia = (uint32_t)gy * (uint32_t)g.W + (uint32_t)xa;
    r.ib = (uint32_t)gy * (uint32_t)g.W + (uint32_t)xb;
    return r;
}
__device__ __forceinline__ float naive_finish(const View& v, const NaivePrep& r, float4 own, float4 fa, float4 fb)
{
    const float w0 = 1.0f - r.w1;
    const float v0 = w0 * fa.x + r.w1 * fb.x, v1 = w0 * fa.y + r.w1 * fb.y, v2 = w0 * fa.z + r.w1 * fb.z, v3 = w0 * fa.w + r.w1 * fb.w;
    const float col = (fabsf(own.x - v0) + fabsf(own.y - v1)) + fabsf(own.z - v2);
    const float grad = fabsf(own.w - v3);
    return ((col < v.th_color) ? col : v.th_color) + ((grad < v.th_grad) ? grad : v.th_grad);
}

__device__ __forceinline__ bool label_valid(const Geom& g, float a, float b, float c, float v, int gx, int gy)
{
    float fx = (float)gx, fy = (float)gy;
    float ds = ((fx * a + fy * b) + 1.0f * c) + 0.0f * v;
    float a5 = a * 5, b5 = b * 5;
    float d;
    return (ds >= g.mind && ds <= g.maxd
            && ((d = ds + a5 + b5) >= g.mind) && d <= g.maxd
            && ((d = ds + a5 - b5) >= g.mind) && d <= g.maxd
            && ((d = ds - a5 + b5) >= g.mind) && d <= g.maxd
            && ((d = ds - a5 - b5) >= g.mind) && d <= g.maxd);
}

__device__ __forceinline__ float guide_centred_f32(uint32_t ipk, int k)
{
    int u = (int)((ipk >> (8 * k)) & 0xffu);
    float w = (float)(2 * u - 255) * (1.0f / 510.0f);
    return k == 3 ? 1.0f : w;
}
__device__ __forceinline__ float guide10_field_f32(uint32_t w10, int off)
{
#if defined(LES_SIM)
    const int v = ((int)(w10 << (22 - off))) >> 22;
#else
    const int v = __builtin_amdgcn_sbfe((int)w10, (unsigned)off, 10u);
#endif
    return (float)v * (1.0f / 510.0f);
}
__device__ __forceinline__ float guide10_centred_f32(uint32_t w10, int k)
{
#if defined(LES_SIM)
    const int v = ((int)(w10 << (22 - 10 * (k < 3 ? k : 0)))) >> 22;
#else
    const int v = __builtin_amdgcn_sbfe((int)w10, (unsigned)(10 * k), 10u);
#endif
    const float w = (float)v * (1.0f / 510.0f);
    return k == 3 ? 1.0f : w;
}
__device__ __forceinline__ double guide_centred_f64(uint32_t ipk, int k)
{
    int u = (int)((ipk >> (8 * k)) & 0xffu);
    double w = fma((double)u, 1.0 / 255, -0.5);
    return k == 3 ? 1.0 : w;
}

__device__ __forceinline__ int window_count(int c, int R, int lo, int hi)
{
    int a = c - R < lo ? lo : c - R;
    int b = c + R + 1 > hi ? hi : c + R + 1;
    return b > a ? b - a : 0;
}

#if defined(LES_SIM)
#define LES_SCHED_FENCE(step) ((void)0)
#else
#define LES_SCHED_FENCE(step) do { if (((step) & 3) == 3) __builtin_amdgcn_sched_barrier(0); } while (0)
#endif
#if defined(LES_SIM)
#define LES_SCHED_FENCE_V(row) ((void)0)
#else
#define LES_SCHED_FENCE_V(row) do { if (((row) % 3) == 2) __builtin_amdgcn_sched_barrier(0); } while (0)
#endif

#ifndef LES_H1_F32
typedef double H1ACC;
#else
typedef float H1ACC;
#endif

template <int V>
struct IntTag { static constexpr int value = V; };

template <int... Is, typename F>
__device__ __forceinline__ void static_for_impl(std::integer_sequence<int, Is...>, F&& f)
{
    (f(IntTag<Is>{}), ...);
}
template <int N, typename F>
__device__ __forceinline__ void static_for(F&& f)
{
    static_for_impl(std::make_integer_sequence<int, N>{}, f);
}

template <int R, int RS>
struct VLane {
    static constexpr int KS = 2 * R + 1;
    static_assert(RS >= KS, "ring shorter than the window");
    float ring1[RS] = {};
    float ring2[RS] = {};
    double S1 = 0.0, S2 = 0.0;
    int k;

    template <int S>
    __device__ __forceinline__ float step(float in, bool keep, double rn1, float4 s)
    {
        constexpr int OLD = (S + RS - KS) % RS;
        S1 += (double)in - (double)ring1[OLD];
        ring1[S] = in;
        const double m = S1 * rn1;
        const double mp = quad_bcast<3>(m);
        const float cov = (float)fma(-(double)s.x, mp, m);
        const float ak = fmaf(s.w, quad_bcast<2>(cov), fmaf(s.z, quad_bcast<1>(cov), s.y * quad_bcast<0>(cov)));
        const float bb = (float)mp - quad_sum(ak * s.x);
        float val = (k < 3) ? ak : bb;
        if (!keep) val = 0.0f;
        S2 += (double)val - (double)ring2[OLD];
        ring2[S] = val;
        return (float)S2;
    }
};

template <int R, int WA, int BY, int SEG>
struct StripCfg {
    static constexpr int TW = WA - 2 * R;
    static constexpr int WP = WA + 2 * R;
    static constexpr int NT = 4 * WA;
    static constexpr int HL = 4 * BY * SEG;
    static constexpr int L1 = (WA + SEG - 1) / SEG;
    static constexpr int L2 = (TW + SEG - 1) / SEG;
    static constexpr int TPITCH = WA * 4 + 4;
    static constexpr int KS = 2 * R + 1;
    static constexpr int RS = ((KS + BY - 1) / BY) * BY;
    static_assert(HL <= NT, "more H lanes than threads");
    static_assert(TW > 0, "strip too narrow for this radius");
};

#if defined(LES_PHASE_TIMING) && !defined(LES_SIM)
__device__ unsigned long long les_dbg[12];
#define LES_PHASE_BEGIN() unsigned long long ph_[5] = {0, 0, 0, 0, 0}; unsigned long long tl_ = clock64()
#define LES_PHASE_MARK(k) do { const unsigned long long now_ = clock64(); ph_[k] += now_ - tl_; tl_ = now_; } while (0)
#define LES_PHASE_END() do { if (threadIdx.x == 0) { for (int k_ = 0; k_ < 5; k_++) atomicAdd(&les_dbg[k_], ph_[k_]); atomicAdd(&les_dbg[5], 1ull); } } while (0)
#else
#define LES_PHASE_BEGIN() ((void)0)
#define LES_PHASE_MARK(k) ((void)0)
#define LES_PHASE_END() ((void)0)
#endif

template <int R, int WA, int BY, int SEG, int MW, int SRC = 0>
__global__ void __launch_bounds__(4 * WA, MW)
les_strip_kernel(Geom g, View view, const Job* __restrict__ jobs, const float4* __restrict__ planes,
                 float* __restrict__ out, int njobs, int check)
{
    using Cfg = StripCfg<R, WA, BY, SEG>;
    constexpr int TW = Cfg::TW, WP = Cfg::WP, NT = Cfg::NT, HL = Cfg::HL, L1 = Cfg::L1, L2 = Cfg::L2;
    constexpr int TPITCH = Cfg::TPITCH, KS = Cfg::KS, RS = Cfg::RS;

    __shared__ float s_p[BY][WP];
    __shared__ uint32_t s_ipk[BY][WP];
    __shared__ float s_T[BY][TPITCH];
    __shared__ uint32_t s_ipk2[BY][TW];
    __shared__ double s_rtab[2 * R + 2];
    __shared__ uint32_t s_c510[WP];
    struct RowInfo { double rny; int flags; uint32_t soff; };
    __shared__ RowInfo s_row[BY];
    struct GRow { uint32_t rowpx; float d_base; };
    __shared__ GRow s_grow[BY];
    __shared__ double s_rnx2[TW + 4];
    __shared__ int s_gsy[BY];
    float (*s_q)[WP] = s_p;

    int job_id;
    {
        const int nwg = (int)gridDim.x, orig = (int)blockIdx.x;
        const int q = nwg / 8, r = nwg % 8, xcd = orig % 8;
        job_id = (xcd < r ? xcd * (q + 1) : r * (q + 1) + (xcd - r) * q) + orig / 8;
    }
    if (job_id >= njobs) return;
    const Job job = jobs[job_id];
    const float4 plane = planes[job.plane_idx];
    const int tid = (int)threadIdx.x;
    const int Ttot = job.th + 4 * R;

    if (tid < 2 * R + 2) s_rtab[tid] = tid > 0 ? 1.0 / (double)tid : 0.0;
    if (tid < WP) s_c510[tid] = 510u;

    const int vx = tid >> 2, vk = tid & 3;
    VLane<R, RS> vl;
    vl.k = vk;
    const int gx1 = job.tx0 - R + vx;
    const bool col_in_clip = gx1 >= job.cx0 && gx1 < job.cx1;
    const int nx1 = window_count(gx1, R, job.cx0, job.cx1);

    const bool h_active = tid < HL;
    const int hk = tid & 3, hrow = (tid >> 2) % BY, hseg = (tid >> 2) / BY;
    const uint32_t* h1_guide = hk < 3 ? &s_ipk[hrow][0] : &s_c510[0];
    const int h1_off = hk < 3 ? 10 * hk : 0;

    __syncthreads();
    const double rnx1 = s_rtab[nx1];

    constexpr int GRP = NT / WP, GPASS = (BY + GRP - 1) / GRP;
    constexpr int ORP = NT / TW, OPASS = (BY + ORP - 1) / ORP;
    const int g_ri = tid / WP, g_xi = tid - g_ri * WP;
    const bool g_lane = tid < GRP * WP;
    const int g_gx = job.tx0 - 2 * R + g_xi;
    const bool g_col_in = g_gx >= job.cx0 && g_gx < job.cx1;
    const int g_sx = min(max(g_gx, job.cx0), job.cx1 - 1);
    const float g_ax = plane.x * (float)g_sx;
    const int o_ri = tid / TW, o_xo = tid - o_ri * TW;
    const bool o_lane = tid < ORP * TW;
    const int o_sx = min(max(job.tx0 + o_xo, job.cx0), job.cx1 - 1);
    const uint32_t HWu = (uint32_t)g.H * (uint32_t)g.W;

    constexpr int PD = (BY % 4 == 0) ? 4 : ((BY % 3 == 0) ? 3 : 1);
    const int sgx1 = min(max(gx1, job.cx0), job.cx1 - 1);
    const float4* st_col = vk < 3 ? view.stats + (size_t)sgx1 * 3 + vk : view.stats + (size_t)g.H * g.W * 3;
    const size_t st_stride = (size_t)g.W * 3;
    auto stats_row = [&](int t) -> float4 {
        const int gy1 = min(max(job.ty0 - 3 * R + t, job.cy0), job.cy1 - 1);
        return st_col[(vk < 3 ? (size_t)gy1 : (size_t)0) * st_stride];
    };
    float4 pre[PD];
#pragma unroll
    for (int j = 0; j < PD; j++) pre[j] = stats_row(j);

    auto fill_row_tables = [&](int tb) {
        const int t = tb + tid;
        const int gy1 = job.ty0 - 3 * R + t;
        RowInfo ri;
        ri.rny = s_rtab[window_count(gy1, R, job.cy0, job.cy1)];
        ri.flags = ((gy1 >= job.cy0 && gy1 < job.cy1) ? 1 : 0) | (t >= 2 * R ? 2 : 0);
        ri.soff = (uint32_t)min(max(gy1 + PD, job.cy0), job.cy1 - 1) * (uint32_t)(g.W * 3);
        s_row[tid] = ri;
        const int gy = job.ty0 - 2 * R + t;
        GRow gr;
        const int sy = min(max(gy, job.cy0), job.cy1 - 1);
        gr.rowpx = ((uint32_t)sy * (uint32_t)g.W) | ((t < Ttot && gy >= job.cy0 && gy < job.cy1) ? 0x80000000u : 0u);
        gr.d_base = plane.y * (float)sy + plane.z;
        s_grow[tid] = gr;
        if constexpr (SRC == 1) s_gsy[tid] = sy;
    };
    if (tid < BY) fill_row_tables(0);
    if (tid < TW + 4) s_rnx2[tid] = s_rtab[window_count(job.tx0 + tid, R, job.cx0, job.cx1)];
    __syncthreads();

    LES_PHASE_BEGIN();
    for (int t0 = 0; t0 < Ttot; t0 += BY) {
        {
            if constexpr (SRC == 1) {
#pragma unroll 1
                for (int jp = 0; jp < GPASS; jp++) {
                    const int i = jp * GRP + g_ri;
                    const GRow gr = s_grow[i < BY ? i : BY - 1];
                    const bool inside = g_lane && g_col_in && i < BY && (gr.rowpx >> 31);
                    const int sy = s_gsy[i < BY ? i : BY - 1];
                    const uint32_t px = (gr.rowpx & 0x7fffffffu) + (uint32_t)g_sx;
                    const NaivePrep np = naive_prepare(g, view.sign, plane.x, plane.y, plane.z, g_sx, sy);
                    const float4 own = view.feat_self[px], fa = view.feat_other[np.ia], fb = view.feat_other[np.ib];
                    const uint32_t ip = view.ipk10[px];
                    if (g_lane && i < BY) {
                        s_p[i][g_xi] = inside ? naive_finish(view, np, own, fa, fb) : 0.0f;
                        s_ipk[i][g_xi] = ip;
                    }
                }
            } else {
                constexpr int GB = 7;
                static_for<(GPASS + GB - 1) / GB>([&](auto btag) {
                    constexpr int J0 = decltype(btag)::value * GB;
                    constexpr int JN = (GPASS - J0) < GB ? (GPASS - J0) : GB;
                    GatherPrep gp[JN];
                    float v0[JN], v1[JN];
                    uint32_t ipa[JN];
#pragma unroll
                    for (int j = 0; j < JN; j++) {
                        const int i = (J0 + j) * GRP + g_ri;
                        const GRow gr = s_grow[i < BY ? i : BY - 1];
                        const bool inside = g_lane && g_col_in && i < BY && (gr.rowpx >> 31);
                        const uint32_t px = (gr.rowpx & 0x7fffffffu) + (uint32_t)g_sx;
                        gp[j] = gather_prepare(g, g_ax, gr.d_base, px, HWu, inside);
                        v0[j] = view.vol[gp[j].i0];
                        v1[j] = view.vol[gp[j].i1];
                        ipa[j] = view.ipk10[px];
                    }
#pragma unroll
                    for (int j = 0; j < JN; j++) {
                        const int i = (J0 + j) * GRP + g_ri;
                        if (g_lane && i < BY) {
                            s_p[i][g_xi] = gather_finish(g, gp[j], v0[j], v1[j]);
                            s_ipk[i][g_xi] = ipa[j];
                        }
                    }
                });
            }
            uint32_t ipo[OPASS];
#pragma unroll
            for (int j = 0; j < OPASS; j++) {
                const int i = j * ORP + o_ri;
                const int sy = min(max(job.ty0 + t0 + i - 4 * R, job.cy0), job.cy1 - 1);
                ipo[j] = view.ipk[(uint32_t)sy * (uint32_t)g.W + (uint32_t)o_sx];
            }
#pragma unroll
            for (int j = 0; j < OPASS; j++) {
                const int i = j * ORP + o_ri;
                if (o_lane && i < BY) s_ipk2[i][o_xo] = ipo[j];
            }
        }
        __syncthreads();
        LES_PHASE_MARK(0);

        if (h_active) {
            float ring[KS];
#pragma unroll
            for (int i = 0; i < KS; i++) ring[i] = 0.0f;
            H1ACC S = 0;
            const int x0 = hseg * L1;
#pragma unroll
            for (int s = 0; s < L1 + 2 * R; s++) {
                const int xi = x0 + s;
                const float f = xi < WP ? guide10_field_f32(h1_guide[xi], h1_off) * s_p[hrow][xi] : 0.0f;
                S += (H1ACC)f - (H1ACC)ring[s % KS];
                ring[s % KS] = f;
                if (s >= 2 * R && x0 + s - 2 * R < WA) s_T[hrow][(x0 + s - 2 * R) * 4 + hk] = (float)S;
                LES_SCHED_FENCE(s);
            }
        }
        __syncthreads();
        LES_PHASE_MARK(1);

        {
            const float* trow = &s_T[0][vx * 4 + vk];
            auto vblock = [&](auto base_tag) {
                constexpr int BASE = decltype(base_tag)::value;
                static_for<BY>([&](auto itag) {
                    constexpr int i = decltype(itag)::value;
                    const RowInfo ri = s_row[i];
                    const double rn1 = rnx1 * ri.rny;
                    const float o = vl.template step<BASE + i>(trow[i * TPITCH], col_in_clip && ri.flags == 3, rn1, pre[i % PD]);
                    pre[i % PD] = st_col[vk < 3 ? ri.soff : 0u];
                    s_T[i][vx * 4 + vk] = o;
                    LES_SCHED_FENCE_V(i);
                });
            };
            const int base = t0 % RS;
            if constexpr (RS / BY == 1) vblock(IntTag<0>{});
            else if constexpr (RS / BY == 2) { if (base == 0) vblock(IntTag<0>{}); else vblock(IntTag<BY>{}); }
            else if constexpr (RS / BY == 3) { if (base == 0) vblock(IntTag<0>{}); else if (base == BY) vblock(IntTag<BY>{}); else vblock(IntTag<2 * BY>{}); }
            else {
                static_assert(RS / BY == 4, "unsupported ring/block ratio");
                if (base == 0) vblock(IntTag<0>{}); else if (base == BY) vblock(IntTag<BY>{});
                else if (base == 2 * BY) vblock(IntTag<2 * BY>{}); else vblock(IntTag<3 * BY>{});
            }
        }
        __syncthreads();
        LES_PHASE_MARK(2);

        if (h_active) {
            const int t = t0 + hrow;
            const bool row_ok = t >= 4 * R && t < Ttot;
            const int gy2 = job.ty0 + t - 4 * R;
            const double rny2 = s_rtab[window_count(gy2, R, job.cy0, job.cy1)];
            float ring[KS];
#pragma unroll
            for (int i = 0; i < KS; i++) ring[i] = 0.0f;
            double S = 0.0;
            const int x0 = hseg * L2;
#pragma unroll
            for (int s = 0; s < L2 + 2 * R; s++) {
                const int xa = x0 + s;
                const float f = xa < WA ? s_T[hrow][xa * 4 + hk] : 0.0f;
                S += (double)f - (double)ring[s % KS];
                ring[s % KS] = f;
                if (s >= 2 * R) {
                    const int xo = x0 + s - 2 * R;
                    const uint32_t ip = xo < TW ? s_ipk2[hrow][xo] : 0u;
                    const double qn = quad_sum(S * guide_centred_f64(ip, hk));
                    const double rn2 = rny2 * s_rnx2[xo < TW + 4 ? xo : TW + 3];
                    const int col = (hk == 0 && xo < TW && row_ok) ? xo : TW + hk;
                    s_q[hrow][col] = (float)(qn * rn2);
                }
                LES_SCHED_FENCE(s);
            }
        }
        __syncthreads();
        LES_PHASE_MARK(3);

        if (tid < BY) fill_row_tables(t0 + BY);
        for (int idx = tid; idx < BY * TW; idx += NT) {
            const int i = idx / TW, xo = idx - i * TW;
            const int t = t0 + i;
            if (t >= 4 * R && t < Ttot && xo < job.tw) {
                const int gy2 = job.ty0 + t - 4 * R, gx2 = job.tx0 + xo;
                float q = s_q[i][xo];
                if (check && !label_valid(g, plane.x, plane.y, plane.z, plane.w, gx2, gy2)) q = LES_COST_INVALID;
                out[job.out_off + (long long)(t - 4 * R) * job.out_stride + xo] = q;
            }
        }
        __syncthreads();
        LES_PHASE_MARK(4);
    }
    LES_PHASE_END();
}

__global__ void les_pack_guide_kernel(const uint8_t* __restrict__ bgr, uint32_t* __restrict__ ipk, uint32_t* __restrict__ ipk10, int P)
{
    int i = (int)(blockIdx.x * blockDim.x + threadIdx.x);
    if (i >= P) return;
    const uint32_t b = bgr[3 * (size_t)i], g = bgr[3 * (size_t)i + 1], r = bgr[3 * (size_t)i + 2];
    ipk[i] = b | (g << 8) | (r << 16);
    ipk10[i] = ((2u * b - 255u) & 1023u) | (((2u * g - 255u) & 1023u) << 10) | (((2u * r - 255u) & 1023u) << 20);
}

__global__ void les_stats_hsum_kernel(const uint32_t* __restrict__ ipk, double* __restrict__ hs, int H, int W, int R)
{
    int x = (int)(blockIdx.x * blockDim.x + threadIdx.x), y = (int)blockIdx.y;
    if (x >= W) return;
    double s[9] = {0, 0, 0, 0, 0, 0, 0, 0, 0};
    for (int dx = -R; dx <= R; dx++) {
        int xx = x + dx;
        if (xx < 0 || xx >= W) continue;
        uint32_t v = ipk[(size_t)y * W + xx];
        double I0 = (double)(v & 0xff) * (1.0 / 255), I1 = (double)((v >> 8) & 0xff) * (1.0 / 255),
               I2 = (double)((v >> 16) & 0xff) * (1.0 / 255);
        s[0] += I0; s[1] += I1; s[2] += I2;
        s[3] += I0 * I0; s[4] += I0 * I1; s[5] += I0 * I2; s[6] += I1 * I1; s[7] += I1 * I2; s[8] += I2 * I2;
    }
    size_t P = (size_t)H * W;
    for (int k = 0; k < 9; k++) hs[k * P + (size_t)y * W + x] = s[k];
}

__global__ void les_stats_finish_kernel(const double* __restrict__ hs, float4* __restrict__ stats, int H, int W, int R, double eps)
{
    int x = (int)(blockIdx.x * blockDim.x + threadIdx.x), y = (int)blockIdx.y;
    if (x >= W) return;
    size_t P = (size_t)H * W;
    double s[9] = {0, 0, 0, 0, 0, 0, 0, 0, 0};
    for (int dy = -R; dy <= R; dy++) {
        int yy = y + dy;
        if (yy < 0 || yy >= H) continue;
        for (int k = 0; k < 9; k++) s[k] += hs[k * P + (size_t)yy * W + x];
    }
    double N = (double)(window_count(x, R, 0, W) * window_count(y, R, 0, H));
    double m0 = s[0] / N, m1 = s[1] / N, m2 = s[2] / N;
    double rr = s[3] / N - m0 * m0 + eps, rg = s[4] / N - m0 * m1, rb = s[5] / N - m0 * m2;
    double gg = s[6] / N - m1 * m1 + eps, gb = s[7] / N - m1 * m2, bb = s[8] / N - m2 * m2 + eps;
    double irr = gg * bb - gb * gb, irg = gb * rb - rg * bb, irb = rg * gb - gg * rb;
    double igg = rr * bb - rb * rb, igb = rb * rg - rr * gb, ibb = rr * gg - rg * rg;
    double det = irr * rr + irg * rg + irb * rb;
    irr /= det; irg /= det; irb /= det; igg /= det; igb /= det; ibb /= det;
    size_t px = (size_t)y * W + x;
    stats[px * 3 + 0] = make_float4((float)(m0 - 0.5), (float)irr, (float)irg, (float)irb);
    stats[px * 3 + 1] = make_float4((float)(m1 - 0.5), (float)irg, (float)igg, (float)igb);
    stats[px * 3 + 2] = make_float4((float)(m2 - 0.5), (float)irb, (float)igb, (float)ibb);
}

__global__ void les_naive_features_kernel(const uint8_t* __restrict__ img, float4* __restrict__ feat, int H, int W, float alpha)
{
    const int x = blockIdx.x * blockDim.x + threadIdx.x, y = blockIdx.y;
    if (x >= W) return;
    auto gray = [&](int xx) {
        const uint8_t* p = img + ((size_t)y * W + xx) * 3;
        return ((float)p[0] * 0.114f + (float)p[1] * 0.587f) + (float)p[2] * 0.299f;
    };
    const float gx = 0.5f * (gray(min(x + 1, W - 1)) - gray(max(x - 1, 0)));
    const uint8_t* p = img + ((size_t)y * W + x) * 3;
    const double k = 1.0 - (double)alpha;
    float4 f;
    f.x = (float)((double)p[0] * k); f.y = (float)((double)p[1] * k); f.z = (float)((double)p[2] * k);
    f.w = gx * alpha;
    feat[(size_t)y * W + x] = f;
}

struct RawCall {
    int fx, fy, fw, fh;
    long long off;
};
__global__ void les_naive_raw_kernel(Geom g, View view, const RawCall* __restrict__ calls, const float4* __restrict__ planes,
                                     float* __restrict__ raw)
{
    const RawCall rc = calls[blockIdx.x];
    const float4 plane = planes[blockIdx.x];
    const long long area = (long long)rc.fw * rc.fh;
    const long long per = (area + gridDim.y - 1) / gridDim.y;
    const long long p0 = per * blockIdx.y, p1 = p0 + per < area ? p0 + per : area;
    for (long long p = p0 + threadIdx.x; p < p1; p += blockDim.x) {
        const int yy = (int)(p / rc.fw), xx = (int)(p - (long long)yy * rc.fw);
        const int gx = rc.fx + xx, gy = rc.fy + yy;
        const NaivePrep np = naive_prepare(g, view.sign, plane.x, plane.y, plane.z, gx, gy);
        const uint32_t px = (uint32_t)gy * (uint32_t)g.W + (uint32_t)gx;
        raw[rc.off + p] = naive_finish(view, np, view.feat_self[px], view.feat_other[np.ia], view.feat_other[np.ib]);
    }
}

__global__ void les_calib_copy_kernel(const float* __restrict__ src, float* __restrict__ dst, size_t n)
{
    const size_t i = (size_t)blockIdx.x * blockDim.x + threadIdx.x;
    if (i < n) dst[i] = src[i];
}

__global__ void les_calib_copy_wide_kernel(const float4* __restrict__ src, float4* __restrict__ dst, size_t n4)
{
    const size_t i = ((size_t)blockIdx.x * 4) * blockDim.x + threadIdx.x;
#pragma unroll
    for (int k = 0; k < 4; k++) {
        const size_t j = i + (size_t)k * blockDim.x;
        if (j < n4) dst[j] = src[j];
    }
}

__global__ void les_fill_out_of_view_kernel(float* __restrict__ vol, int D, int H, int W, int mode)
{
    const int x = (int)(blockIdx.x * blockDim.x + threadIdx.x), y = (int)blockIdx.y, d = (int)blockIdx.z;
    float* row = vol + ((size_t)d * H + y) * W;
    if (mode == 0) {
        const int q = d < W - 1 ? d : W - 1;
        if (x < q) row[x] = row[q];
    } else {
        int p = W - d;
        if (p < 1) p = 1;
        if (x >= p && x < W) row[x] = row[p - 1];
    }
}

__global__ void les_convert_l2r_kernel(const float* __restrict__ src, float* __restrict__ dst, int D, int H, int W)
{
    const int x = (int)(blockIdx.x * blockDim.x + threadIdx.x), y = (int)blockIdx.y, d = (int)blockIdx.z;
    if (x >= W) return;
    const float* s0 = src + ((size_t)d * H + y) * W;
    float v;
    if (d >= W) v = s0[x];
    else v = x < W - 1 - d ? s0[x + d] : s0[W - 1];
    dst[((size_t)d * H + y) * W + x] = v;
}

struct WtaJob { int x, y, w, h; };

__global__ void les_wta_kernel(const WtaJob* __restrict__ jobs, const float4* __restrict__ planes,
                               float* __restrict__ cur_cost, const float* __restrict__ prop_cost,
                               float4* __restrict__ labels, int W)
{
    const WtaJob j = jobs[blockIdx.x];
    const float4 pl = planes[blockIdx.x];
    for (int idx = (int)(blockIdx.y * blockDim.x + threadIdx.x); idx < j.w * j.h; idx += (int)(blockDim.x * gridDim.y)) {
        int yy = idx / j.w, xx = idx - yy * j.w;
        size_t k = (size_t)(j.y + yy) * W + j.x + xx;
        float pc = prop_cost[k];
        if (cur_cost[k] > pc) {
            cur_cost[k] = pc;
            labels[k] = pl;
        }
    }
}

struct XchgRect { int x, y, w, h; int off; int rank; };

__global__ void les_xchg_pack_kernel(const XchgRect* __restrict__ rects, int first, const float4* __restrict__ labels,
                                     const float* __restrict__ cost, float* __restrict__ slot, int lmax, int W)
{
    const XchgRect r = rects[first + blockIdx.x];
    float4* sl = reinterpret_cast<float4*>(slot);
    float* sc = slot + 4 * (size_t)lmax;
    for (int idx = (int)(blockIdx.y * blockDim.x + threadIdx.x); idx < r.w * r.h; idx += (int)(blockDim.x * gridDim.y)) {
        const int yy = idx / r.w, xx = idx - yy * r.w;
        const size_t k = (size_t)(r.y + yy) * W + r.x + xx;
        sl[r.off + idx] = labels[k];
        sc[r.off + idx] = cost[k];
    }
}

__global__ void les_xchg_unpack_kernel(const XchgRect* __restrict__ rects, const float* __restrict__ recv, float4* __restrict__ labels,
                                       float* __restrict__ cost, int lmax, int W, int own_rank)
{
    const XchgRect r = rects[blockIdx.x];
    if (r.rank == own_rank) return;
    const float* slot = recv + 5 * (size_t)lmax * (size_t)r.rank;
    const float4* sl = reinterpret_cast<const float4*>(slot);
    const float* sc = slot + 4 * (size_t)lmax;
    for (int idx = (int)(blockIdx.y * blockDim.x + threadIdx.x); idx < r.w * r.h; idx += (int)(blockDim.x * gridDim.y)) {
        const int yy = idx / r.w, xx = idx - yy * r.w;
        const size_t k = (size_t)(r.y + yy) * W + r.x + xx;
        labels[k] = sl[r.off + idx];
        cost[k] = sc[r.off + idx];
    }
}

}
```

localexpstereo_amd/csrc/les_march.h:

```cpp
#pragma once

#include "les_kernels.h"

#if defined(LES_MARCH_LAB)
#include "les_march_lab.h"
#else
#define LES_MARCH_ROLE_ORDER 5
#define LES_STATS_POLICY ""
#define LES_LAB_ROLE_ON(bit) true
#define LES_LAB_ABLATE(bit) false
#endif
#ifndef LES_TICK_BEGIN
#define LES_TICK_BEGIN() ((void)0)
#define LES_TICK_MARK() ((void)0)
#define LES_TICK_BARRIER() __syncthreads()
#define LES_TICK_END(role_) ((void)0)
#endif

namespace les {

constexpr int kMarchSH = 5;
constexpr int kMarchMB = 24;
constexpr int kMarchSL = 3;
constexpr int kMarchS2 = 4;
constexpr int kMarchMagicBits = 0x4B400000;
static_assert(kMarchSH + kMarchMB + kMarchSL == 32, "N cov = t - hi32(M * (s << SL)) needs the scales to meet at 2^32");
__host__ __device__ constexpr int march_pb(int R) { return (2 * R + 1) * (2 * R + 1) < 512 ? 20 : 19; }
#ifndef LES_MARCH_STAT_WORDS
#define LES_MARCH_STAT_WORDS 9
#endif
constexpr int kMarchStatWords = LES_MARCH_STAT_WORDS;
static_assert(kMarchStatWords == 9 || kMarchStatWords == 12, "statistics record of 36 or 48 bytes");

struct MarchView {
    const float* vol;
    const uint32_t* ipk8;
    const float* mstats;
    float sp;
    float pmagic;
    float poff;
    float kapS;
    float upS;
    float qscale;
    float kmu;
    const long long* raw_off;
    const float* vol_t;
};
#ifndef LES_TILED_MIN_SLOPE_WIDE
#define LES_TILED_MIN_SLOPE_WIDE 0.05f
#endif
#ifndef LES_TILED_MIN_SLOPE
#define LES_TILED_MIN_SLOPE 0.125f
#endif

template <int R, int WGC, int NJ, int BY>
struct MarchCfg {
    static constexpr int KS = 2 * R + 1;
    static constexpr int RS = 3 * BY;
    static constexpr int TW = WGC - 4 * R;
    static constexpr int HWV = WGC / 64;
    static constexpr int NW = 3 * HWV * NJ;
    static constexpr int NT = 64 * NW;
    static constexpr int SEGL = 8;
    static constexpr int PADW = 16;
    static constexpr int PCOLS0 = 1 + WGC + WGC / PADW;
    static constexpr int PCOLS = PCOLS0 + ((4 - PCOLS0 % 8) + 8) % 8;
    static_assert(RS >= KS, "the ring must hold a whole window (the row that leaves it is the one written KS rows ago)");
    static_assert(RS - KS < BY, "a ring longer than the window by a block or more wastes registers: pick the smallest block height");
    static_assert(WGC % 64 == 0, "a job slot is a whole number of waves");
    static_assert(BY * (64 / SEGL) <= 64, "one wave prefixes its own tile");
    static_assert(TW > 0, "job too narrow for this radius");
    static_assert(2 * R + 1 < 64, "a window crosses at most one wave boundary");
    static_assert((long long)KS * KS * (1ll << (march_pb(R) - 1 + kMarchSL)) < (1ll << 31), "stage-1 window sums (shifted for the product with M) must fit int32");
    static_assert((long long)KS * 128 * (1ll << (march_pb(R) - 1)) < (1ll << 31), "vertical sums of Iq * pi must fit int32");
    static_assert((long long)KS * (1ll << (30 - kMarchS2)) < (1ll << 31), "the stage-2 window sums, rounded to 2^S2, must fit int32");
    __host__ __device__ static constexpr int pcol(int ci) { return 1 + ci + ci / PADW; }
};

__device__ __forceinline__ void march_prefix_scan8(int4 (&v)[8])
{
#pragma unroll
    for (int j = 1; j < 8; j++) { v[j].x += v[j - 1].x; v[j].y += v[j - 1].y; v[j].z += v[j - 1].z; v[j].w += v[j - 1].w; }
    int4 inc = v[7];
#if defined(LES_SIM) || defined(LES_MARCH_SCAN_PLAIN)
#define LES_SCAN_STEP(N) { inc.x += dpp_row_shr<N>(inc.x); inc.y += dpp_row_shr<N>(inc.y); inc.z += dpp_row_shr<N>(inc.z); inc.w += dpp_row_shr<N>(inc.w); }
    LES_SCAN_STEP(2) LES_SCAN_STEP(4) LES_SCAN_STEP(8)
#undef LES_SCAN_STEP
#else
#define LES_SCAN_ROW(N) "v_add_u32_dpp %0, %0, %0 row_shr:" #N " row_mask:0xf bank_mask:0xf bound_ctrl:1\n" \
                        "v_add_u32_dpp %1, %1, %1 row_shr:" #N " row_mask:0xf bank_mask:0xf bound_ctrl:1\n" \
                        "v_add_u32_dpp %2, %2, %2 row_shr:" #N " row_mask:0xf bank_mask:0xf bound_ctrl:1\n" \
                        "v_add_u32_dpp %3, %3, %3 row_shr:" #N " row_mask:0xf bank_mask:0xf bound_ctrl:1\n"
    asm("s_nop 1\n" LES_SCAN_ROW(2) LES_SCAN_ROW(4) LES_SCAN_ROW(8) : "+v"(inc.x), "+v"(inc.y), "+v"(inc.z), "+v"(inc.w));
#undef LES_SCAN_ROW
#endif
    const int4 off = int4{inc.x - v[7].x, inc.y - v[7].y, inc.z - v[7].z, inc.w - v[7].w};
#pragma unroll
    for (int j = 0; j < 8; j++) { v[j].x += off.x; v[j].y += off.y; v[j].z += off.z; v[j].w += off.w; }
}

template <int BY, int PCOLS>
__device__ __forceinline__ void march_prefix_tile(int4 (*T)[PCOLS], int ci0, int lane)
{
    constexpr int SEGL = 8;
    const int row = 2 * (lane >> 4) + (lane & 1), seg = (lane & 15) >> 1;
    const bool act = row < BY;
    const int c0 = ci0 + seg * SEGL;
    int4* p = &T[act ? row : 0][1 + c0 + c0 / 16];
    int4 v[SEGL];
#pragma unroll
    for (int j = 0; j < SEGL; j++) v[j] = p[j];
    march_prefix_scan8(v);
    if (act) {
#pragma unroll
        for (int j = 0; j < SEGL; j++) lds_store4(&p[j], v[j].x, v[j].y, v[j].z, v[j].w);
    }
}

template <int BY, int PCOLS>
__device__ __forceinline__ void march_prefix_pair(int4 (*TA)[PCOLS], int4 (*TB)[PCOLS], int ci0, int lane)
{
    constexpr int SEGL = 8;
    const int row = 2 * (lane >> 4) + (lane & 1), seg = (lane & 15) >> 1;
    const bool act = row < BY;
    const int c0 = ci0 + seg * SEGL;
    const int pc = 1 + c0 + c0 / 16;
    int4* pa = &TA[act ? row : 0][pc];
    int4* pb = &TB[act ? row : 0][pc];
    int4 va[SEGL], vb[SEGL];
#pragma unroll
    for (int j = 0; j < SEGL; j++) vb[j] = pb[j];
    wave_sync();
#pragma unroll
    for (int j = 0; j < SEGL; j++) va[j] = pa[j];
    LES_MARCH_SCHED_FENCE();
    march_prefix_scan8(vb);
    if (act) {
#pragma unroll
        for (int j = 0; j < SEGL; j++) lds_store4(&pb[j], vb[j].x, vb[j].y, vb[j].z, vb[j].w);
    }
    LES_MARCH_SCHED_FENCE();
    march_prefix_scan8(va);
    if (act) {
#pragma unroll
        for (int j = 0; j < SEGL; j++) lds_store4(&pa[j], va[j].x, va[j].y, va[j].z, va[j].w);
    }
}

#if defined(LES_SIM)
typedef float4 mstat4;
#else
typedef float mstat4 __attribute__((ext_vector_type(4)));
#endif
#if LES_MARCH_STAT_WORDS == 9
typedef float mstat_tail;
#else
typedef mstat4 mstat_tail;
#endif
struct MarchStatRow { mstat4 a, b; mstat_tail c; };
#if defined(LES_SIM) || defined(LES_MARCH_STATS_PLAIN)
struct MarchStatDesc { const char* base; uint32_t bytes; };
__device__ inline MarchStatDesc march_stats_desc(const float* base, uint32_t bytes) { return MarchStatDesc{(const char*)base, bytes}; }
__device__ inline void march_stats_load(MarchStatRow& r, const MarchStatDesc& d, uint32_t voff, uint32_t soff)
{
    const unsigned long long o = (unsigned long long)voff + (unsigned long long)soff;
    float w[8 + sizeof(mstat_tail) / 4];
    for (unsigned i = 0; i < sizeof w / 4; i++) w[i] = (o + 4ull * i + 4 <= d.bytes) ? *reinterpret_cast<const float*>(d.base + o + 4ull * i) : 0.0f;
    memcpy(&r.a, w, 16); memcpy(&r.b, w + 4, 16); memcpy(&r.c, w + 8, sizeof r.c);
}
template <int N>
__device__ inline void march_stats_wait(MarchStatRow& r) { (void)r; }
template <int N>
__device__ inline void march_stats_wait(MarchStatRow& r, MarchStatRow& q) { (void)r; (void)q; }
#else
typedef int MarchStatDesc __attribute__((ext_vector_type(4)));
__device__ __forceinline__ MarchStatDesc march_stats_desc(const float* base, uint32_t bytes)
{
    const unsigned long long a = (unsigned long long)base;
    MarchStatDesc d;
    d.x = __builtin_amdgcn_readfirstlane((int)(uint32_t)a);
    d.y = __builtin_amdgcn_readfirstlane((int)((uint32_t)(a >> 32) & 0xffffu));
    d.z = __builtin_amdgcn_readfirstlane((int)bytes);
    d.w = 0x00027000;
    return d;
}
__device__ __forceinline__ void march_stats_load(MarchStatRow& r, const MarchStatDesc& d, uint32_t voff, uint32_t soff)
{
    asm volatile("buffer_load_dwordx4 %0, %1, %2, %3 offen" LES_STATS_POLICY : "+v"(r.a) : "v"(voff), "s"(d), "s"(soff));
    asm volatile("buffer_load_dwordx4 %0, %1, %2, %3 offen offset:16" LES_STATS_POLICY : "+v"(r.b) : "v"(voff), "s"(d), "s"(soff));
#if LES_MARCH_STAT_WORDS == 9
    asm volatile("buffer_load_dword %0, %1, %2, %3 offen offset:32" LES_STATS_POLICY : "+v"(r.c) : "v"(voff), "s"(d), "s"(soff));
#else
    asm volatile("buffer_load_dwordx4 %0, %1, %2, %3 offen offset:32" LES_STATS_POLICY : "+v"(r.c) : "v"(voff), "s"(d), "s"(soff));
#endif
}
template <int N>
__device__ __forceinline__ void march_stats_wait(MarchStatRow& r) { asm volatile("s_waitcnt vmcnt(%3)" : "+v"(r.a), "+v"(r.b), "+v"(r.c) : "n"(N)); }
template <int N>
__device__ __forceinline__ void march_stats_wait(MarchStatRow& r, MarchStatRow& q)
{
    asm volatile("s_waitcnt vmcnt(%6)" : "+v"(r.a), "+v"(r.b), "+v"(r.c), "+v"(q.a), "+v"(q.b), "+v"(q.c) : "n"(N));
}
#endif
__device__ __forceinline__ int march_stat_m2(const MarchStatRow& r)
{
#if LES_MARCH_STAT_WORDS == 9
    return __float_as_int(r.c);
#else
    return __float_as_int(r.c.x);
#endif
}

__device__ __forceinline__ bool march_label_surely_valid(const Geom& g, float4 pl, int x0, int x1, int y0, int y1)
{
    const float ax0 = pl.x * (float)x0, ax1 = pl.x * (float)x1, by0 = pl.y * (float)y0, by1 = pl.y * (float)y1;
    const float spread = 5.0f * (fabsf(pl.x) + fabsf(pl.y));
    const float lo = (fminf(ax0, ax1) + fminf(by0, by1)) + pl.z - spread;
    const float hi = (fmaxf(ax0, ax1) + fmaxf(by0, by1)) + pl.z + spread;
    const float mag = fmaxf(fabsf(ax0), fabsf(ax1)) + fmaxf(fabsf(by0), fabsf(by1)) + fabsf(pl.z) + spread;
    const float margin = 1e-5f * mag + 1e-30f;
    return (0.0f * pl.w == 0.0f) && mag < 1e30f && (lo - margin >= g.mind) && (hi + margin <= g.maxd);
}

__device__ __forceinline__ bool march_plane_short_gather(const Geom& g, float4 pl, const Job& job, int R, int* slice_lo)
{
    *slice_lo = 0;
    const unsigned long long HW = (unsigned long long)g.H * (unsigned long long)g.W;
    const bool moderate = fabsf(pl.x) < 1e30f && fabsf(pl.y) < 1e30f && fabsf(pl.z) < 1e30f;
    if (!(moderate && g.mind == 0.0f && g.D0 == 0 && g.maxd == (float)(g.D - 1) && g.D >= 2 && HW < (1ull << 24))) return false;
    if ((unsigned long long)g.D * HW < (1ull << 30)) return true;
    const int x0 = max(job.tx0 - 2 * R, job.cx0), x1 = min(job.tx0 + job.tw + 2 * R, job.cx1) - 1;
    const int y0 = max(job.ty0 - 2 * R, job.cy0), y1 = min(job.ty0 + job.th + 2 * R, job.cy1) - 1;
    if (x1 < x0 || y1 < y0) return false;
    const float ax0 = pl.x * (float)x0, ax1 = pl.x * (float)x1, by0 = pl.y * (float)y0, by1 = pl.y * (float)y1;
    const float lo = (fminf(ax0, ax1) + fminf(by0, by1)) + pl.z, hi = (fmaxf(ax0, ax1) + fmaxf(by0, by1)) + pl.z;
    const float mag = fmaxf(fabsf(ax0), fabsf(ax1)) + fmaxf(fabsf(by0), fabsf(by1)) + fabsf(pl.z);
    const float margin = 1e-5f * mag + 1e-30f;
    if (!((lo - margin >= 0.0f) && (hi + margin < g.maxd))) return false;
    const int s0 = (int)floorf(lo - margin), s1 = (int)floorf(hi + margin) + 1;
    *slice_lo = s0;
    return s0 >= 0 && s1 < g.D && (unsigned long long)(s1 - s0 + 1) * HW < (1ull << 28);
}

template <int R, int WGC, int NJ, int BY>
__global__ void __launch_bounds__(3 * WGC * NJ)
les_march_kernel(Geom g, MarchView view, const Job* __restrict__ jobs, const float4* __restrict__ planes,
                 float* __restrict__ out, int ngroups, int check)
{
    using Cfg = MarchCfg<R, WGC, NJ, BY>;
    constexpr int KS = Cfg::KS, RS = Cfg::RS, NT = Cfg::NT, HWV = Cfg::HWV, PCOLS = Cfg::PCOLS;
    constexpr int UN = 3;

    __shared__ int4 s_T1[2][NJ][BY][PCOLS];
    __shared__ int4 s_T2[3][NJ][BY][PCOLS];
    __shared__ float s_rtab[KS + 1];

    int grp;
    {
        const int nwg = (int)gridDim.x, orig = (int)blockIdx.x;
        const int q = nwg / 8, r = nwg % 8, xcd = orig % 8;
        grp = (xcd < r ? xcd * (q + 1) : r * (q + 1) + (xcd - r) * q) + orig / 8;
    }
    if (grp >= ngroups) return;
    const int tid = (int)threadIdx.x;
    const int lane = tid & 63;
    const int wave = readfirstlane_i32(tid >> 6);
    constexpr int kRoleOf[6][3] = {{0, 1, 2}, {2, 1, 0}, {1, 2, 0}, {2, 0, 1}, {1, 0, 2}, {0, 2, 1}};
    const int slot = wave / (3 * HWV), role = kRoleOf[LES_MARCH_ROLE_ORDER][(wave % (3 * HWV)) / HWV], half = wave % HWV;
    const int ci0 = half * 64, ci = ci0 + lane;
    const Job job = jobs[grp * NJ + slot];
    int th_max = 0;
#pragma unroll
    for (int s = 0; s < NJ; s++) th_max = max(th_max, jobs[grp * NJ + s].th);
    const int nblk = (th_max + 4 * R + BY - 1) / BY;
    const int nticks = nblk + 3;
    const int Ttot = job.th > 0 ? job.th + 4 * R : 0;
    const float4 plane = planes[job.plane_idx];
    const int cy1m = max(job.cy1 - 1, job.cy0);

    if (tid <= KS) s_rtab[tid] = tid > 0 ? (float)(1.0 / (double)tid) : 0.0f;
    for (int k = tid; k < 3 * NJ * BY; k += NT) {
        if (k < 2 * NJ * BY) (&s_T1[0][0][0][0])[k * PCOLS] = int4{0, 0, 0, 0};
        (&s_T2[0][0][0][0])[k * PCOLS] = int4{0, 0, 0, 0};
    }
    __syncthreads();

    const int gx = job.tx0 - 2 * R + ci;
    const bool col_in = gx >= job.cx0 && gx < job.cx1 && job.th > 0;
    const int sx = min(max(gx, job.cx0), max(job.cx1 - 1, job.cx0));
    const uint32_t sx4 = (uint32_t)sx * 4u;
    const uint32_t rowB = (uint32_t)g.W * 4u;
    const uint32_t imgB = (uint32_t)g.H * rowB;
    const BufRsrc rs_guide = make_buf(view.ipk8, imgB);
    const int nx = window_count(gx, R, job.cx0, job.cx1);
    const int cP = min(ci + R, WGC - 1), cM = ci - R - 1;
    const int pcP = Cfg::pcol(cP);
    const int pcM = cM >= 0 ? Cfg::pcol(cM) : 0;
    const bool cross = cM >= 0 && (cP >> 6) != (cM >> 6);
    const int pcX = cross ? Cfg::pcol((cP >> 6) * 64 - 1) : 0;
    const int pcS = Cfg::pcol(ci);

    if (role == 0 && LES_LAB_ROLE_ON(1)) {
        const uint32_t HWu = (uint32_t)g.H * (uint32_t)g.W;
        const float g_ax = plane.x * (float)sx;
        const bool fronto = plane.x == 0.0f && plane.y == 0.0f;
        GatherPrep gpc = gather_prepare(g, 0.0f, plane.z, 0u, HWu, true);
        if (gpc.f1 == 0.0f) gpc.i1 = gpc.i0;
        int ringN[RS];
        uint32_t ringG[RS];
#pragma unroll
        for (int k = 0; k < RS; k++) { ringN[k] = 0; ringG[k] = 0u; }
        int Sp = 0;
        int Sc[3] = {1 << (kMarchSH - 1), 1 << (kMarchSH - 1), 1 << (kMarchSH - 1)};
        const uint32_t i0s = (uint32_t)readfirstlane_i32((int)gpc.i0), i1s = (uint32_t)readfirstlane_i32((int)gpc.i1);
        const float f1s = __int_as_float(readfirstlane_i32(__float_as_int(gpc.f1)));
        const int modes = readfirstlane_i32(gpc.mode);
        const float f0s = 1.0f - f1s;
        const bool inv_job = fronto && modes == 2 && !view.raw_off;
        int slice_lo = 0;
        const bool tame = !fronto && !view.raw_off && march_plane_short_gather(g, plane, job, R, &slice_lo);
        const uint32_t W8 = ((uint32_t)g.W + 7u) >> 3;
        const uint32_t trowB = W8 * (uint32_t)g.D * 32u;
        const int trow_lo = max(job.ty0 - 2 * R, job.cy0);
        const int trow_hi = min(job.ty0 - 2 * R + (nblk + 2) * BY, job.cy1);
        const unsigned long long tspanB = (unsigned long long)max(trow_hi - trow_lo, 1) * (unsigned long long)trowB;
        const bool tiled = tame && view.vol_t && fabsf(plane.x) >= (NJ == 1 ? LES_TILED_MIN_SLOPE_WIDE : LES_TILED_MIN_SLOPE) && tspanB < 0xfffffff0ull &&
                           (unsigned long long)W8 * (unsigned long long)g.D * 32ull < (1ull << 31);
        const float spj = !col_in ? 0.0f : (inv_job ? 0.0f : view.sp);
        const float pmj = !col_in ? __int_as_float(kMarchMagicBits) : (inv_job ? fmaf(g.th_col, view.sp, view.pmagic) : view.pmagic);
        auto march_a = [&](auto kind_tag) __attribute__((always_inline)) {
        constexpr int KIND = decltype(kind_tag)::value;
        GatherPrep gp[BY];
        float v0[BY], v1[BY];
        float f1r[BY];
        uint32_t gw[BY];
        uint32_t rowbits = 0, rowbits_nx = 0;
        int nx_rowB = 0;
        float nx_dbase = 0.0f;
        int nx_rowraw = 0;
        int nx_rowT = 0;
        const int fw = job.cx1 - job.cx0;
        const float* v0base = view.vol + (size_t)i0s;
        if constexpr (KIND == 3) v0base = view.vol + view.raw_off[job.plane_idx] - job.cx0;
        if constexpr (KIND == 4) v0base = view.vol + (size_t)slice_lo * (size_t)HWu;
        if constexpr (KIND == 5) v0base = view.vol_t + (size_t)trow_lo * (size_t)(trowB >> 2);
        const unsigned long long rest4 = (unsigned long long)(g.D - slice_lo) * (unsigned long long)imgB;
        const unsigned long long trestB = (unsigned long long)(g.H - trow_lo) * (unsigned long long)trowB;
        const uint32_t tiledB = (uint32_t)(trestB < 0xfffffffcull ? trestB : 0xfffffffcull);
        const BufRsrc rs_v0 = make_buf(v0base, KIND == 3 ? 0xfffffffcu : (KIND == 4 ? (uint32_t)(rest4 < 0xfffffffcull ? rest4 : 0xfffffffcull) : (KIND == 5 ? tiledB : imgB)));
        const uint32_t tcol = (((uint32_t)sx >> 3) * (uint32_t)g.D * 8u + ((uint32_t)sx & 7u)) * 4u;
        const int dsub = g.D0 - slice_lo;
        const BufRsrc rs_v1 = make_buf(view.vol + (size_t)i1s, imgB);
        auto prep = [&](int b) __attribute__((always_inline)) {
            const int t = b * BY + lane;
            const int gy = job.ty0 - 2 * R + t;
            const int sy = min(max(gy, job.cy0), cy1m);
            nx_rowB = (int)((uint32_t)sy * rowB);
            rowbits_nx = ballot_low(t < Ttot && gy >= job.cy0 && gy < job.cy1, BY);
            if constexpr (KIND == 3) nx_rowraw = (sy - job.cy0) * fw * 4;
            else nx_dbase = plane.y * (float)sy + plane.z;
            if constexpr (KIND == 5) nx_rowT = (int)((uint32_t)(sy - trow_lo) * trowB);
        };
        auto issue_row = [&](auto itag) __attribute__((always_inline)) {
            constexpr int i = decltype(itag)::value;
            const uint32_t ro = (uint32_t)readlane_i32(nx_rowB, i);
            if (LES_LAB_ABLATE(64)) { v0[i] = (float)lane; v1[i] = 0.0f; gw[i] = (uint32_t)lane; return; }
            if constexpr (KIND == 3) {
                v0[i] = buf_load<float>(rs_v0, sx4, (uint32_t)readlane_i32(nx_rowraw, i));
            } else if constexpr (KIND < 2) {
                v0[i] = buf_load<float>(rs_v0, sx4, ro);
                if constexpr (KIND == 1) v1[i] = buf_load<float>(rs_v1, sx4, ro);
            } else if constexpr (KIND == 4) {
                const float d = g_ax + readlane_f32(nx_dbase, i);
                const float dc = med3_f32(d, 0.0f, g.maxd);
                const float df = floorf(dc);
                f1r[i] = dc - df;
                const uint32_t e = mad_u24((int)df + dsub, (int)HWu, sx);
                v0[i] = buf_load<float>(rs_v0, e << 2, ro);
                v1[i] = buf_load<float>(rs_v0, (e << 2) + (f1r[i] > 0.0f ? imgB : 0u), ro);
            } else if constexpr (KIND == 5) {
                const float d = g_ax + readlane_f32(nx_dbase, i);
                const float dc = med3_f32(d, 0.0f, g.maxd);
                const float df = floorf(dc);
                f1r[i] = dc - df;
                const uint32_t e = (((uint32_t)(int)df + (uint32_t)g.D0) << 5) + tcol;
                const uint32_t rt = (uint32_t)readlane_i32(nx_rowT, i);
                v0[i] = buf_load<float>(rs_v0, e, rt);
                v1[i] = buf_load<float>(rs_v0, e + (f1r[i] > 0.0f ? 32u : 0u), rt);
            } else {
                const float d_base = readlane_f32(nx_dbase, i);
                const bool inside = col_in && ((rowbits_nx >> i) & 1u);
                gp[i] = gather_prepare(g, g_ax, d_base, (ro >> 2) + (uint32_t)sx, HWu, inside);
                if (gp[i].f1 == 0.0f) gp[i].i1 = gp[i].i0;
                v0[i] = view.vol[gp[i].i0];
                v1[i] = view.vol[gp[i].i1];
            }
            gw[i] = buf_load<uint32_t>(rs_guide, sx4, ro);
        };
        prep(0);
        rowbits = rowbits_nx;
        prep(0);
        static_for<BY>([&](auto itag) { issue_row(itag); });
        LES_TICK_BEGIN();
        for (int k0 = 0; k0 < nticks; k0 += UN) {
            static_for<UN>([&](auto utag) {
                constexpr int BASE = decltype(utag)::value * BY;
                const int k = k0 + decltype(utag)::value;
                if (k < nticks) {
                    if (k < nblk) {
                        int4 (*T)[PCOLS] = s_T1[k & 1][slot];
                        prep(k + 1);
                        static_for<BY>([&](auto itag) {
                            constexpr int i = decltype(itag)::value;
                            constexpr int SLOT = BASE + i;
                            constexpr int OLD = (SLOT + RS - KS) % RS;
                            int pi;
                            if constexpr (KIND == 3) {
                                pi = (__float_as_int(fmaf(v0[i], spj, pmj)) - kMarchMagicBits) & sbfe1(rowbits, i);
                            } else if constexpr (KIND < 2) {
                                float C = v0[i];
                                if constexpr (KIND == 1) C = f0s * v0[i] + f1s * v1[i];
                                const float p = min_f32_finite(C, g.th_col);
                                pi = (__float_as_int(fmaf(p, spj, pmj)) - kMarchMagicBits) & sbfe1(rowbits, i);
                            } else if constexpr (KIND == 4 || KIND == 5) {
                                const float f0 = 1.0f - f1r[i];
                                const float C = f0 * v0[i] + f1r[i] * v1[i];
                                const float p = min_f32_finite(C, g.th_col);
                                pi = (__float_as_int(fmaf(p, spj, pmj)) - kMarchMagicBits) & sbfe1(rowbits, i);
                            } else {
                                const float p = gather_finish(g, gp[i], v0[i], v1[i]);
                                pi = __float_as_int(fmaf(p, view.sp, view.pmagic)) - kMarchMagicBits;
                                pi = gp[i].mode == 3 ? 0 : pi;
                            }
                            const uint32_t gi = gw[i];
                            const int no = ringN[OLD];
                            const uint32_t go = ringG[OLD];
                            ringN[SLOT] = -pi;
                            ringG[SLOT] = gi;
                            Sp = Sp + pi + no;
                            Sc[0] = Sc[0] + mul24_sbyte<0>(gi, pi) + mul24_sbyte<0>(go, no);
                            Sc[1] = Sc[1] + mul24_sbyte<1>(gi, pi) + mul24_sbyte<1>(go, no);
                            Sc[2] = Sc[2] + mul24_sbyte<2>(gi, pi) + mul24_sbyte<2>(go, no);
                            lds_store4(&T[i][pcS], Sp, Sc[0] >> kMarchSH, Sc[1] >> kMarchSH, Sc[2] >> kMarchSH);
                            issue_row(itag);
                        });
                        rowbits = rowbits_nx;
                        LES_TICK_MARK();
                    }
                    {
                        int4 (*TB)[PCOLS] = s_T2[(decltype(utag)::value + UN - 2 % UN) % UN][slot];
                        const bool da = k < nblk, db = !(NJ > 1 && KIND == 2) && k >= 2 && k < nblk + 2;
                        constexpr bool kPair = KIND != 2 && KIND != 4 && KIND != 5;
                        if (kPair && da && db) march_prefix_pair<BY, PCOLS>(s_T1[k & 1][slot], TB, ci0, lane);
                        else {
                            if (da) { wave_sync(); march_prefix_tile<BY, PCOLS>(s_T1[k & 1][slot], ci0, lane); }
                            if (db) march_prefix_tile<BY, PCOLS>(TB, ci0, lane);
                        }
                    }
                    LES_TICK_BARRIER();
                }
            });
        }
        LES_TICK_END(0);
        };
        if (view.raw_off) march_a(std::integral_constant<int, 3>{});
        else if (fronto && f1s == 0.0f) march_a(std::integral_constant<int, 0>{});
        else if (fronto) march_a(std::integral_constant<int, 1>{});
        else if (tiled) march_a(std::integral_constant<int, 5>{});
        else if (tame) march_a(std::integral_constant<int, 4>{});
        else march_a(std::integral_constant<int, 2>{});
    } else if (role == 1 && LES_LAB_ROLE_ON(2)) {
        const bool s1_col = col_in && ci >= R && ci < WGC - R;
        int slice_lo_unused = 0;
        const bool general_plane = !view.raw_off && !(plane.x == 0.0f && plane.y == 0.0f) && !march_plane_short_gather(g, plane, job, R, &slice_lo_unused);
        const float kap_x = s1_col ? view.kapS * s_rtab[nx] : 0.0f;
        const float up_x = s1_col ? view.upS * s_rtab[nx] : 0.0f;
        const uint32_t sxS = (uint32_t)sx * (uint32_t)(4 * kMarchStatWords);
        const uint32_t rowS = (uint32_t)g.W * (uint32_t)(4 * kMarchStatWords);
        const MarchStatDesc ds_stats = march_stats_desc(view.mstats, (uint32_t)g.H * rowS);
        MarchStatRow st[BY];
#pragma unroll
        for (int i = 0; i < BY; i++) {
            st[i].a = st[i].b = mstat4{0.0f, 0.0f, 0.0f, 0.0f};
#if LES_MARCH_STAT_WORDS == 9
            st[i].c = 0.0f;
#else
            st[i].c = mstat4{0.0f, 0.0f, 0.0f, 0.0f};
#endif
        }
        float rny[BY];
        int nx_srow = 0;
        float nx_rny = 0.0f;
        auto prep = [&](int b) __attribute__((always_inline)) {
            const int t = b * BY + lane;
            const int gy1 = job.ty0 - 3 * R + t;
            const bool on = gy1 >= job.cy0 && gy1 < job.cy1 && t >= 2 * R && t < Ttot;
            nx_rny = on ? s_rtab[window_count(gy1, R, job.cy0, job.cy1)] : 0.0f;
            nx_srow = (int)((uint32_t)min(max(gy1, job.cy0), cy1m) * rowS);
        };
        auto issue_row = [&](auto itag) __attribute__((always_inline)) {
            constexpr int i = decltype(itag)::value;
            rny[i] = readlane_f32(nx_rny, i);
            uint32_t soff = (uint32_t)readlane_i32(nx_srow, i) & 0xfffffffcu;
            if (LES_LAB_ABLATE(4)) soff &= 0x3u;
            if (LES_LAB_ABLATE(1)) return;
            march_stats_load(st[i], ds_stats, sxS, soff);
        };
        prep(0);
        static_for<BY>([&](auto itag) { issue_row(itag); });
        LES_TICK_BEGIN();
        for (int k = 0; k < nticks; k++) {
            if (k >= 1 && k <= nblk) {
                const int b = k - 1;
                const int4 (*T1)[PCOLS] = s_T1[b & 1][slot];
                int4 (*T2)[PCOLS] = s_T2[b % 3][slot];
                constexpr int GC = 2, NS = (BY + GC - 1) / GC;
                prep(k);
                int4 pp[2][GC], pm[2][GC], px[2][GC];
                auto lds_stage = [&](auto stag) __attribute__((always_inline)) {
                    constexpr int S = decltype(stag)::value;
#pragma unroll
                    for (int j = 0; j < GC; j++)
                        if (S * GC + j < BY) {
                            if (LES_LAB_ABLATE(2)) { pp[S & 1][j] = int4{lane, k, 2, 3}; pm[S & 1][j] = int4{3, 2, k, lane}; px[S & 1][j] = int4{0, 0, 0, 0}; }
                            else { pp[S & 1][j] = T1[S * GC + j][pcP]; pm[S & 1][j] = T1[S * GC + j][pcM]; px[S & 1][j] = T1[S * GC + j][pcX]; }
                        }
                };
                lds_stage(std::integral_constant<int, 0>{});
                static_for<NS>([&](auto gtag) {
                    constexpr int S = decltype(gtag)::value, CB = S & 1;
                    constexpr int LO = S * GC;
                    constexpr int N = (BY - LO) < GC ? (BY - LO) : GC;
                    if constexpr (S + 1 < NS) lds_stage(std::integral_constant<int, S + 1>{});
                    LES_MARCH_SCHED_FENCE();
                    static_assert(GC == 2, "vmcnt bookkeeping below is written for stages of two rows");
                    if constexpr (N == 2) march_stats_wait<3 * (BY - 2)>(st[LO], st[LO + 1]);
                    else march_stats_wait<3 * (BY - 1)>(st[LO]);
                    static_for<N>([&](auto jtag) {
                        constexpr int j = decltype(jtag)::value;
                        constexpr int i = LO + j;
                        const int s = pp[CB][j].x - pm[CB][j].x + px[CB][j].x;
                        const mstat4 q0 = st[i].a, q1 = st[i].b;
                        const int M0 = __float_as_int(q1.z), M1 = __float_as_int(q1.w), M2 = march_stat_m2(st[i]);
                        const long long s8 = (long long)(s << kMarchSL);
                        const float d0 = (float)((pp[CB][j].y - pm[CB][j].y) + px[CB][j].y + (int)(((long long)M0 * s8 + (1ll << 31)) >> 32));
                        const float d1 = (float)((pp[CB][j].z - pm[CB][j].z) + px[CB][j].z + (int)(((long long)M1 * s8 + (1ll << 31)) >> 32));
                        const float d2 = (float)((pp[CB][j].w - pm[CB][j].w) + px[CB][j].w + (int)(((long long)M2 * s8 + (1ll << 31)) >> 32));
                        const float ka = kap_x * rny[i];
                        const float a0 = fmaf(q0.z, d2, fmaf(q0.y, d1, q0.x * d0)) * ka;
                        const float a1 = fmaf(q1.x, d2, fmaf(q0.w, d1, q0.y * d0)) * ka;
                        const float a2 = fmaf(q1.y, d2, fmaf(q1.x, d1, q0.z * d0)) * ka;
                        const float mp = (float)s * (up_x * rny[i]);
#if LES_MARCH_STAT_WORDS == 9
                        const float bb = fmaf(view.kmu, fmaf(a2, (float)M2, fmaf(a1, (float)M1, a0 * (float)M0)), mp);
#else
                        const float bb = fmaf(-a2, st[i].c.w, fmaf(-a1, st[i].c.z, fmaf(-a0, st[i].c.y, mp)));
#endif
                        lds_store4(&T2[i][pcS], cvt_rpi_i32(a0), cvt_rpi_i32(a1), cvt_rpi_i32(a2), cvt_rpi_i32(bb));
                    });
                    LES_MARCH_SCHED_FENCE();
                    static_for<N>([&](auto jtag) { issue_row(std::integral_constant<int, LO + decltype(jtag)::value>{}); });
                });
                LES_TICK_MARK();
            }
            if (NJ > 1 && general_plane && k >= 2 && k < nblk + 2) march_prefix_tile<BY, PCOLS>(s_T2[(k - 2) % 3][slot], ci0, lane);
            LES_TICK_BARRIER();
        }
        LES_TICK_END(1);
    } else if (role == 2 && LES_LAB_ROLE_ON(4)) {
        const bool out_col = ci >= 2 * R && ci < 2 * R + job.tw && job.th > 0;
        const uint32_t oc4 = (uint32_t)max(ci - 2 * R, 0) * 4u;
        const float vl_xa = (float)gx * plane.x, vl_c = 1.0f * plane.z, vl_zv = 0.0f * plane.w, vl_a5 = plane.x * 5, vl_b5 = plane.y * 5;
        const float c_lane = view.qscale * s_rtab[nx];
        int ring2[4][RS];
#pragma unroll
        for (int k = 0; k < RS; k++) ring2[0][k] = ring2[1][k] = ring2[2][k] = ring2[3][k] = 0;
        long long S2[4] = {1ll << (kMarchS2 - 1), 1ll << (kMarchS2 - 1), 1ll << (kMarchS2 - 1), 1ll << (kMarchS2 - 1)};
        uint32_t gq[BY];
        float rny2[BY];
        uint32_t okbits = 0;
        int nx_grow = 0;
        float nx_rny = 0.0f;
        const BufRsrc rs_out = make_buf(out + job.out_off, 0xfffffffcu);
        const uint32_t ostrideB = (uint32_t)job.out_stride * 4u;
        auto prep = [&](int b) __attribute__((always_inline)) {
            const int t = b * BY + lane;
            const int gy2 = job.ty0 - 4 * R + t;
            nx_rny = s_rtab[window_count(gy2, R, job.cy0, job.cy1)];
            nx_grow = (int)((uint32_t)min(max(gy2, job.cy0), cy1m) * rowB);
            okbits = ballot_low(t >= 4 * R && t < Ttot, BY);
        };
        auto issue_row = [&](auto itag) __attribute__((always_inline)) {
            constexpr int i = decltype(itag)::value;
            rny2[i] = readlane_f32(nx_rny, i);
            if (LES_LAB_ABLATE(128)) { gq[i] = (uint32_t)lane; return; }
            gq[i] = buf_load<uint32_t>(rs_guide, sx4, (uint32_t)readlane_i32(nx_grow, i));
        };
        auto march_d = [&](auto check_tag) __attribute__((always_inline)) {
        constexpr bool CHECK = decltype(check_tag)::value != 0;
        LES_TICK_BEGIN();
        for (int k0 = 0; k0 < nticks; k0 += UN) {
            static_for<UN>([&](auto utag) {
                constexpr int U = decltype(utag)::value;
                constexpr int BASE = ((U + UN - 3 % UN) % UN) * BY;
                const int k = k0 + U;
                if (k < nticks) {
                    if (k >= 3) {
                        const int b = k - 3;
                        const int4 (*T2)[PCOLS] = s_T2[(U + UN - 3 % UN) % UN][slot];
                        constexpr int GD = 1, NS = (BY + GD - 1) / GD;
                        int4 pp[2][GD], pm[2][GD], px[2][GD];
                        auto lds_stage = [&](auto stag) __attribute__((always_inline)) {
                            constexpr int S = decltype(stag)::value;
#pragma unroll
                            for (int j = 0; j < GD; j++)
                                if (S * GD + j < BY) {
                                    if (LES_LAB_ABLATE(16)) { pp[S & 1][j] = int4{lane, b, 2, 3}; pm[S & 1][j] = int4{3, 2, b, lane}; px[S & 1][j] = int4{0, 0, 0, 0}; }
                                    else { pp[S & 1][j] = T2[S * GD + j][pcP]; pm[S & 1][j] = T2[S * GD + j][pcM]; px[S & 1][j] = T2[S * GD + j][pcX]; }
                                }
                        };
                        lds_stage(std::integral_constant<int, 0>{});
                        static_for<NS>([&](auto gtag) {
                            constexpr int S = decltype(gtag)::value, CB = S & 1;
                            constexpr int LO = S * GD;
                            constexpr int N = (BY - LO) < GD ? (BY - LO) : GD;
                            if constexpr (S + 1 < NS) lds_stage(std::integral_constant<int, S + 1>{});
                            LES_MARCH_SCHED_FENCE();
                            static_for<N>([&](auto jtag) {
                                constexpr int j = decltype(jtag)::value;
                                constexpr int i = LO + j;
                                constexpr int SLOT = BASE + i, OLD = (SLOT + RS - KS) % RS;
                                const int h0 = pp[CB][j].x - pm[CB][j].x + px[CB][j].x, h1 = pp[CB][j].y - pm[CB][j].y + px[CB][j].y;
                                const int h2 = pp[CB][j].z - pm[CB][j].z + px[CB][j].z, h3 = pp[CB][j].w - pm[CB][j].w + px[CB][j].w;
                                const int o0 = ring2[0][OLD], o1 = ring2[1][OLD], o2 = ring2[2][OLD], o3 = ring2[3][OLD];
                                ring2[0][SLOT] = h0; ring2[1][SLOT] = h1; ring2[2][SLOT] = h2; ring2[3][SLOT] = h3;
                                acc64_add_i32(S2[0], h0 - o0); acc64_add_i32(S2[1], h1 - o1); acc64_add_i32(S2[2], h2 - o2); acc64_add_i32(S2[3], h3 - o3);
                                if (out_col && ((okbits >> i) & 1u)) {
                                    const int t = b * BY + i;
                                    const uint32_t gi = gq[i];
                                    const float f0 = (float)(int)(S2[0] >> kMarchS2), f1 = (float)(int)(S2[1] >> kMarchS2), f2 = (float)(int)(S2[2] >> kMarchS2), f3 = (float)(int)(S2[3] >> kMarchS2);
                                    const float acc = fmaf(f2, cvt_f32_sbyte<2>(gi), fmaf(f1, cvt_f32_sbyte<1>(gi), fmaf(f0, cvt_f32_sbyte<0>(gi), f3 * 255.0f)));
                                    float q = fmaf(acc * c_lane, rny2[i], view.poff);
                                    if constexpr (CHECK) {
                                        const int gy2 = job.ty0 + t - 4 * R;
                                        const float ds = ((vl_xa + (float)gy2 * plane.y) + vl_c) + vl_zv;
                                        const float dp = ds + vl_a5, dm = ds - vl_a5;
                                        const float d1 = dp + vl_b5, d2 = dp - vl_b5, d3 = dm + vl_b5, d4 = dm - vl_b5;
                                        const float mn = fmin3(fmin3(ds, d1, d2), d3, d4), mx = fmax3(fmax3(ds, d1, d2), d3, d4);
                                        if (!(mn >= g.mind && mx <= g.maxd)) q = LES_COST_INVALID;
                                    }
                                    if (!(LES_LAB_ABLATE(128) && q != 12345.0f))
                                    buf_store<float>(rs_out, oc4, (uint32_t)(t - 4 * R) * ostrideB, q);
                                }
                            });
                            LES_MARCH_SCHED_FENCE();
                        });
                    }
                    if (k >= 2 && k <= nblk + 1) {
                        prep(k - 2);
                        static_for<BY>([&](auto itag) { issue_row(itag); });
                    }
                    LES_TICK_BARRIER();
                }
            });
        }
        LES_TICK_END(2);
        };
        const bool surely_valid = march_label_surely_valid(g, plane, job.tx0, job.tx0 + max(job.tw, 1) - 1, job.ty0, job.ty0 + max(job.th, 1) - 1);
        if (check && !surely_valid) march_d(std::integral_constant<int, 1>{});
        else march_d(std::integral_constant<int, 0>{});
    }
}

__global__ void les_march_stats_kernel(const double* __restrict__ hs, const uint32_t* __restrict__ ipk, uint32_t* __restrict__ ipk8,
                                       float* __restrict__ mstats, unsigned* __restrict__ inv_diag_max, int H, int W, int R, double eps)
{
    int x = (int)(blockIdx.x * blockDim.x + threadIdx.x), y = (int)blockIdx.y;
    if (x >= W) return;
    size_t P = (size_t)H * W;
    double s[9] = {0, 0, 0, 0, 0, 0, 0, 0, 0};
    for (int dy = -R; dy <= R; dy++) {
        int yy = y + dy;
        if (yy < 0 || yy >= H) continue;
        for (int k = 0; k < 9; k++) s[k] += hs[k * P + (size_t)yy * W + x];
    }
    double N = (double)(window_count(x, R, 0, W) * window_count(y, R, 0, H));
    double m0 = s[0] / N, m1 = s[1] / N, m2 = s[2] / N;
    double rr = s[3] / N - m0 * m0 + eps, rg = s[4] / N - m0 * m1, rb = s[5] / N - m0 * m2;
    double gg = s[6] / N - m1 * m1 + eps, gb = s[7] / N - m1 * m2, bb = s[8] / N - m2 * m2 + eps;
    double irr = gg * bb - gb * gb, irg = gb * rb - rg * bb, irb = rg * gb - gg * rb;
    double igg = rr * bb - rb * rb, igb = rb * rg - rr * gb, ibb = rr * gg - rg * rg;
    double det = irr * rr + irg * rg + irb * rb;
    irr /= det; irg /= det; irb /= det; igg /= det; igb /= det; ibb /= det;
    size_t px = (size_t)y * W + x;
    const double fs = (double)(1ll << kMarchMB);
    const double c0 = m0 * 255.0 - 128.0, c1 = m1 * 255.0 - 128.0, c2 = m2 * 255.0 - 128.0;
    const int M0 = (int)fmin(fmax(rint(-c0 * fs), -2147483648.0), 2147483647.0);
    const int M1 = (int)fmin(fmax(rint(-c1 * fs), -2147483648.0), 2147483647.0);
    const int M2 = (int)fmin(fmax(rint(-c2 * fs), -2147483648.0), 2147483647.0);
    float* o = mstats + px * kMarchStatWords;
    o[0] = (float)irr; o[1] = (float)irg; o[2] = (float)irb; o[3] = (float)igg;
    o[4] = (float)igb; o[5] = (float)ibb; o[6] = __int_as_float(M0); o[7] = __int_as_float(M1);
    o[8] = __int_as_float(M2);
    if (kMarchStatWords == 12) { o[9] = (float)(c0 / 255.0); o[10] = (float)(c1 / 255.0); o[11] = (float)(c2 / 255.0); }
    const uint32_t v = ipk[px];
    const uint32_t b0 = ((v & 0xffu) - 128u) & 0xffu, b1 = (((v >> 8) & 0xffu) - 128u) & 0xffu, b2 = (((v >> 16) & 0xffu) - 128u) & 0xffu;
    ipk8[px] = b0 | (b1 << 8) | (b2 << 16);
    const float dmax = fmaxf(fmaxf((float)irr, (float)igg), (float)ibb);
    if (dmax > 0.0f) atomicMax(inv_diag_max, __float_as_uint(dmax));
}

__global__ void les_tile_volume_kernel(const float* __restrict__ src, float* __restrict__ dst, int D, int H, int W)
{
    const int x = (int)(blockIdx.x * 64 + (threadIdx.x & 63)), y = (int)blockIdx.y;
    const int W8 = (W + 7) >> 3;
    if (x >= W8 * 8) return;
    const size_t HW = (size_t)H * W;
    float* o = dst + (((size_t)y * W8 + (size_t)(x >> 3)) * D) * 8 + (x & 7);
    for (int d = (int)(threadIdx.x >> 6); d < D; d += (int)(blockDim.x >> 6))
        o[(size_t)d * 8] = x < W ? src[(size_t)d * HW + (size_t)y * W + x] : 0.0f;
}

__global__ void les_range_kernel(const float* __restrict__ v, size_t n, float* __restrict__ part_min, int* __restrict__ part_bad)
{
    __shared__ float s_min[256];
    __shared__ int s_bad[256];
    float m = INFINITY;
    int bad = 0;
    for (size_t i = (size_t)blockIdx.x * blockDim.x + threadIdx.x; i < n; i += (size_t)gridDim.x * blockDim.x) {
        const float x = v[i];
        if (!(fabsf(x) < INFINITY)) bad = 1;
        else m = fminf(m, x);
    }
    s_min[threadIdx.x] = m; s_bad[threadIdx.x] = bad;
    __syncthreads();
    for (int k = 128; k > 0; k >>= 1) {
        if ((int)threadIdx.x < k) {
            s_min[threadIdx.x] = fminf(s_min[threadIdx.x], s_min[threadIdx.x + k]);
            s_bad[threadIdx.x] |= s_bad[threadIdx.x + k];
        }
        __syncthreads();
    }
    if (threadIdx.x == 0) { part_min[blockIdx.x] = s_min[0]; part_bad[blockIdx.x] = s_bad[0]; }
}

}
```

localexpstereo_amd/csrc/les_march_lab.h:

```cpp
#pragma once

#ifndef LES_MARCH_ROLE_MASK
#define LES_MARCH_ROLE_MASK 7
#endif
#ifndef LES_MARCH_ROLE_ORDER
#define LES_MARCH_ROLE_ORDER 5
#endif
#ifndef LES_MARCH_EXP
#define LES_MARCH_EXP 0
#endif
#ifndef LES_STATS_POLICY
#define LES_STATS_POLICY ""
#endif

#define LES_LAB_ROLE_ON(bit) ((LES_MARCH_ROLE_MASK & (bit)) != 0)
#define LES_LAB_ABLATE(bit) ((LES_MARCH_EXP & (bit)) != 0)

#if defined(LES_PHASE_TIMING) && !defined(LES_SIM)
#define LES_TICK_BEGIN() unsigned long long tk_c_ = 0, tk_w_ = 0, tk_n_ = 0, tk_r_ = 0, tk_m_ = 0, tk_t_ = clock64()
#define LES_TICK_MARK() (tk_m_ = clock64())
#define LES_TICK_BARRIER() do { const unsigned long long a_ = clock64(); __syncthreads(); const unsigned long long b_ = clock64(); tk_c_ += a_ - tk_t_; tk_r_ += (tk_m_ > tk_t_ ? tk_m_ : a_) - tk_t_; tk_w_ += b_ - a_; tk_t_ = b_; tk_n_++; } while (0)
#define LES_TICK_END(role_) do { if (lane == 0) { atomicAdd(&les_dbg[2 * (role_)], tk_c_); atomicAdd(&les_dbg[2 * (role_) + 1], tk_w_); atomicAdd(&les_dbg[6 + (role_)], tk_n_); atomicAdd(&les_dbg[9 + (role_)], tk_r_); } } while (0)
#endif
```

Before: 168,100.

## Chain consecutive column strips through one march workgroup to amortize pipeline fill

Adds a chained mode to the march kernel for NJ==1 entries. One workgroup processes several horizontally adjacent strips in sequence, and each role switches to the next strip's columns at a computed period boundary, so the vertical pipeline's warm-up and drain are paid once per chain rather than once per strip. The host picks the chain length with a cost model over CU count and ticks, and a rotation spreads the start strips. In exchange some parallelism is lost when chains are long, the kernel signature and job layout get more complex, and the debug tick counters are extended.

```diff
diff --git a/localexpstereo_amd/csrc/les_hip.hip b/localexpstereo_amd/csrc/les_hip.hip
--- a/localexpstereo_amd/csrc/les_hip.hip
+++ b/localexpstereo_amd/csrc/les_hip.hip
@@ -116,6 +116,7 @@
     les::Job* d_mjobs = nullptr;
     const MarchEntry* mentry = nullptr;
     int nmgroups = 0;
+    int mchain = 0;
     bool march_ok = false;
     les::RawCall* d_rawcalls = nullptr;
     long long* d_raw_off = nullptr;
@@ -148,7 +149,7 @@
     hipStream_t stream = nullptr;
     float* d_tile = nullptr; float* h_tile = nullptr; size_t tile_cap = 0;
     float4* d_plane = nullptr; float4* h_plane = nullptr;
-    struct Entry { les_hip_rect f, t; int want_march; const void* march; int njobs, ngroups; les::Job* d_jobs; unsigned long long stamp; };
+    struct Entry { les_hip_rect f, t; int want_march; const void* march; int njobs, ngroups, chain; les::Job* d_jobs; unsigned long long stamp; };
     float* d_raw = nullptr; size_t raw_cap = 0;
     les::RawCall* d_rawcall = nullptr; long long* d_raw_off = nullptr;
     les_hip_rect raw_f = {-1, -1, -1, -1};
diff --git a/localexpstereo_amd/csrc/les_hip_batch.inc b/localexpstereo_amd/csrc/les_hip_batch.inc
--- a/localexpstereo_amd/csrc/les_hip_batch.inc
+++ b/localexpstereo_amd/csrc/les_hip_batch.inc
@@ -41,14 +41,14 @@
     {
         std::vector<les::Job> mjobs;
         bool mok = false;
-        build_march_jobs(c, n, frs, trs, out_slabs, mjobs, mok, b->mentry);
+        build_march_jobs(c, n, frs, trs, out_slabs, mjobs, mok, b->mentry, b->mchain);
         if (mok && !mjobs.empty()) {
             if (hipMalloc((void**)&b->d_mjobs, mjobs.size() * sizeof(les::Job)) != hipSuccess ||
                 hipMemcpy(b->d_mjobs, mjobs.data(), mjobs.size() * sizeof(les::Job), hipMemcpyHostToDevice) != hipSuccess) {
                 les_hip_batch_destroy(b);
                 return fail(LES_HIP_ERR_DEVICE, "upload of the march job table failed");
             }
-            b->nmgroups = (int)(mjobs.size() / b->mentry->NJ);
+            b->nmgroups = (int)(mjobs.size() / (b->mchain ? b->mchain : b->mentry->NJ));
             b->march_ok = true;
         }
         if (b->march_ok && c->naive) {
@@ -217,13 +217,13 @@
         d_planes = c->d_planes;
     }
     if (b->march_ok && mode >= 0 && mode <= 1 && c->march && c->v[mode].march_ok) {
-        if (!c->naive) return launch_march(c, b->mentry, mode, b->d_mjobs, b->nmgroups, d_planes, out_dev, check, cur_stream(c));
+        if (!c->naive) return launch_march(c, b->mentry, mode, b->d_mjobs, b->nmgroups, b->mchain, d_planes, out_dev, check, cur_stream(c));
         {
             std::lock_guard<std::mutex> lk(c->mu);
             if (!b->d_raw[mode]) HIPCHECK(hipMalloc((void**)&b->d_raw[mode], (size_t)std::max<long long>(b->raw_floats, 1) * sizeof(float)));
         }
         const RawPatches rp{b->d_rawcalls, b->d_raw_off, b->d_raw[mode], b->n, b->raw_chunks};
-        return launch_march(c, b->mentry, mode, b->d_mjobs, b->nmgroups, d_planes, out_dev, check, cur_stream(c), &rp);
+        return launch_march(c, b->mentry, mode, b->d_mjobs, b->nmgroups, b->mchain, d_planes, out_dev, check, cur_stream(c), &rp);
     }
     return launch_strips(c, mode, b->d_jobs, b->njobs, d_planes, out_dev, check, cur_stream(c));
 }
@@ -302,18 +302,20 @@
         std::vector<les::Job> jobs;
         bool mok = false;
         const MarchEntry* me = nullptr;
-        if (want_march) build_march_jobs(c, 1, fr, tr, 0, jobs, mok, me);
+        int chain = 0;
+        if (want_march) build_march_jobs(c, 1, fr, tr, 0, jobs, mok, me, chain);
         const bool use_march = want_march && mok && !jobs.empty();
         if (!use_march) {
             rc = build_jobs(c, 1, fr, tr, 0, jobs);
             if (rc) return rc;
             me = nullptr;
+            chain = 0;
         }
         for (auto& j : jobs) {
             j.out_off = (long long)(j.ty0 - tr->y) * tr->w + (j.tx0 - tr->x);
             j.out_stride = tr->w;
         }
-        les_hip_scratch::Entry ne{*fr, *tr, want_march, me, (int)jobs.size(), me ? (int)(jobs.size() / me->NJ) : 0, nullptr, 0};
+        les_hip_scratch::Entry ne{*fr, *tr, want_march, me, (int)jobs.size(), me ? (int)(jobs.size() / (chain ? chain : me->NJ)) : 0, chain, nullptr, 0};
         if (s->cache.size() >= 16) {
             size_t k = 0;
             for (size_t i = 1; i < s->cache.size(); i++) if (s->cache[i].stamp < s->cache[k].stamp) k = i;
@@ -367,9 +369,9 @@
             s->raw_f = *fr;
         }
         const RawPatches rp{s->d_rawcall, s->d_raw_off, s->d_raw, 1, (int)std::min<size_t>(1024, (rneed + 4095) / 4096)};
-        rc = launch_march(c, static_cast<const MarchEntry*>(e->march), mode, e->d_jobs, e->ngroups, s->d_plane, s->d_tile, check, s->stream, &rp);
-    }
-    else if (e->march) rc = launch_march(c, static_cast<const MarchEntry*>(e->march), mode, e->d_jobs, e->ngroups, s->d_plane, s->d_tile, check, s->stream);
+        rc = launch_march(c, static_cast<const MarchEntry*>(e->march), mode, e->d_jobs, e->ngroups, e->chain, s->d_plane, s->d_tile, check, s->stream, &rp);
+    }
+    else if (e->march) rc = launch_march(c, static_cast<const MarchEntry*>(e->march), mode, e->d_jobs, e->ngroups, e->chain, s->d_plane, s->d_tile, check, s->stream);
     else rc = launch_strips(c, mode, e->d_jobs, e->njobs, s->d_plane, s->d_tile, check, s->stream);
     if (rc) return rc;
     HIPCHECK(hipMemcpyAsync(s->h_tile, s->d_tile, need * sizeof(float), hipMemcpyDeviceToHost, s->stream));
diff --git a/localexpstereo_amd/csrc/les_hip_context.inc b/localexpstereo_amd/csrc/les_hip_context.inc
--- a/localexpstereo_amd/csrc/les_hip_context.inc
+++ b/localexpstereo_amd/csrc/les_hip_context.inc
@@ -6,8 +6,8 @@
 int les_hip_debug_phases(unsigned long long* out)
 {
     (void)hipDeviceSynchronize();
-    if (hipMemcpyFromSymbol(out, HIP_SYMBOL(les::les_dbg), 12 * sizeof(unsigned long long)) != hipSuccess) return 1;
-    unsigned long long z[12] = {0, 0, 0, 0, 0, 0, 0, 0, 0, 0, 0, 0};
+    if (hipMemcpyFromSymbol(out, HIP_SYMBOL(les::les_dbg), 16 * sizeof(unsigned long long)) != hipSuccess) return 1;
+    unsigned long long z[16] = {0, 0, 0, 0, 0, 0, 0, 0, 0, 0, 0, 0, 0, 0, 0, 0};
     (void)hipMemcpyToSymbol(HIP_SYMBOL(les::les_dbg), z, sizeof z);
     return 0;
 }
diff --git a/localexpstereo_amd/csrc/les_hip_march.inc b/localexpstereo_amd/csrc/les_hip_march.inc
--- a/localexpstereo_amd/csrc/les_hip_march.inc
+++ b/localexpstereo_amd/csrc/les_hip_march.inc
@@ -50,11 +50,12 @@
 }
 
 bool build_march_jobs(les_hip_ctx* c, int n, const les_hip_rect* frs, const les_hip_rect* trs, int out_slabs,
-                      std::vector<les::Job>& jobs, bool& ok, const MarchEntry*& entry)
+                      std::vector<les::Job>& jobs, bool& ok, const MarchEntry*& entry, int& chain)
 {
     jobs.clear();
     ok = false;
     entry = nullptr;
+    chain = 0;
     if (!c->march) return true;
     const int R = c->R, W = c->p.W, H = c->p.H;
     const long long P = (long long)H * W;
@@ -73,8 +74,8 @@
     const MarchEntry* cands[2] = {c->march, find_march(c->R, 0)};
     const MarchEntry* m = c->march;
     int max_rows = 1 << 30;
+    double best = 1e300;
     {
-        double best = 1e300;
         const int row_opts[] = {1 << 30, 1024, 512, 384, 256, 192, 128, 96, 64, 48, 32};
         for (int g = 0; g < 2; g++) {
             const MarchEntry* e = cands[g];
@@ -100,8 +101,62 @@
             }
         }
     }
+    const MarchEntry* w = cands[0];
+    const char* ce = getenv("LES_HIP_MARCH_CHAIN");
+    const int force = ce ? atoi(ce) : -1;
+    bool chainable = w && w->NJ == 1 && force != 0 && !getenv("LES_HIP_MARCH_ROWS") &&
+                     (c->naive || (unsigned long long)c->p.D * (unsigned long long)P < (1ull << 30));
+    if (const char* e = getenv("LES_HIP_MARCH_WIDE")) if (atoi(e) == 0) chainable = false;
+    int max_ns = 0, th_max = 0;
+    for (int i = 0; i < n && chainable; i++) {
+        const les_hip_rect &f = frs[i], &t = trs[i];
+        if (t.w <= 0 || t.h <= 0) continue;
+        if (t.y != f.y || t.h != f.h) chainable = false;
+        max_ns = std::max(max_ns, (t.w + w->TW - 1) / w->TW);
+        th_max = std::max(th_max, t.h);
+    }
+    if (chainable && max_ns > 0) {
+        int pick = 0;
+        for (int L = 1; L <= max_ns; L++) {
+            long long chains = 0;
+            for (int i = 0; i < n; i++)
+                if (trs[i].w > 0 && trs[i].h > 0) chains += ((trs[i].w + w->TW - 1) / w->TW + L - 1) / L;
+            const int Pd = les::march_chain_period(th_max, R, w->BY);
+            const double ticks = (double)(((long long)(L - 1) * Pd + th_max + 2 * R + w->BY - 1) / w->BY + 3);
+            const double cost = (double)((chains + ncu - 1) / ncu) * ticks * (1.0 + 1e-3 * (double)chains / ncu);
+            if (force > 0 ? L == std::min(force, max_ns) : cost < best) { best = cost; pick = L; }
+        }
+        if (pick > 0) { m = w; max_rows = 1 << 30; chain = pick; }
+    }
     if (const char* e = getenv("LES_HIP_MARCH_ROWS")) max_rows = std::max(1, atoi(e));
     entry = m;
+    if (chain) {
+        const int TW = m->TW;
+        long long nchains = 0, ci = 0;
+        for (int i = 0; i < n; i++)
+            if (trs[i].w > 0 && trs[i].h > 0) nchains += ((trs[i].w + TW - 1) / TW + chain - 1) / chain;
+        for (int i = 0; i < n; i++) {
+            const les_hip_rect &f = frs[i], &t = trs[i];
+            if (t.w <= 0 || t.h <= 0) continue;
+            const int ns = (t.w + TW - 1) / TW, sw = (t.w + ns - 1) / ns;
+            for (int s0 = 0; s0 < ns; s0 += chain, ci++) {
+                const int len = std::min(chain, ns - s0), rot = len == ns ? (int)((ci * 8 / std::max(nchains, 1ll)) % ns) : 0;
+                for (int s = s0; s < s0 + chain; s++) {
+                    les::Job j;
+                    const int sx = (s < s0 + len ? s0 + (s - s0 + rot) % len : ns - 1) * sw;
+                    j.tx0 = t.x + sx; j.ty0 = t.y;
+                    j.tw = std::min(sw, t.w - sx); j.th = t.h;
+                    j.cx0 = f.x; j.cy0 = f.y; j.cx1 = f.x + f.w; j.cy1 = f.y + f.h;
+                    j.out_off = (out_slabs ? (long long)(i / out_slabs) * P : 0) + (long long)j.ty0 * W + j.tx0;
+                    j.out_stride = W;
+                    j.plane_idx = i;
+                    if (s >= ns) { j.tw = 0; j.th = 0; }
+                    jobs.push_back(j);
+                }
+            }
+        }
+        return true;
+    }
     const int TW = m->TW, NJ = m->NJ;
     for (int i = 0; i < n; i++) {
         const les_hip_rect &f = frs[i], &t = trs[i];
@@ -153,7 +208,7 @@
     return view;
 }
 
-int launch_march(les_hip_ctx* c, const MarchEntry* m, int mode, const les::Job* d_mjobs, int ngroups, const float4* d_planes, float* d_out, int check,
+int launch_march(les_hip_ctx* c, const MarchEntry* m, int mode, const les::Job* d_mjobs, int ngroups, int chain, const float4* d_planes, float* d_out, int check,
                  hipStream_t stream, const RawPatches* rp = nullptr)
 {
     if (ngroups <= 0) return LES_HIP_OK;
@@ -163,7 +218,7 @@
         hipLaunchKernelGGL(les::les_naive_raw_kernel, dim3(rp->n, rp->chunks), dim3(256), 0, stream, c->geom, strip_view(c, mode), rp->calls, d_planes, rp->raw);
         mv.vol = rp->raw; mv.raw_off = rp->off;
     }
-    hipLaunchKernelGGL(m->fn, dim3(ngroups), dim3(m->NT), 0, stream, c->geom, mv, d_mjobs, d_planes, d_out, ngroups, check);
+    hipLaunchKernelGGL(m->fn, dim3(ngroups), dim3(m->NT), 0, stream, c->geom, mv, d_mjobs, d_planes, d_out, ngroups, check, chain);
     HIPCHECK(hipGetLastError());
     return LES_HIP_OK;
 }
diff --git a/localexpstereo_amd/csrc/les_hip_march_tables.inc b/localexpstereo_amd/csrc/les_hip_march_tables.inc
--- a/localexpstereo_amd/csrc/les_hip_march_tables.inc
+++ b/localexpstereo_amd/csrc/les_hip_march_tables.inc
@@ -36,7 +36,7 @@
     return def;
 }
 
-typedef void (*MarchKernel)(les::Geom, les::MarchView, const les::Job*, const float4*, float*, int, int);
+typedef void (*MarchKernel)(les::Geom, les::MarchView, const les::Job*, const float4*, float*, int, int, int);
 struct MarchEntry { int R; int TW; int NJ; int NT; int BY; MarchKernel fn; };
 #define LES_MARCH_ENTRY(R_, WGC_, NJ_, BY_) \
     { R_, les::MarchCfg<R_, WGC_, NJ_, BY_>::TW, NJ_, les::MarchCfg<R_, WGC_, NJ_, BY_>::NT, BY_, les::les_march_kernel<R_, WGC_, NJ_, BY_> }
diff --git a/localexpstereo_amd/csrc/les_kernels.h b/localexpstereo_amd/csrc/les_kernels.h
--- a/localexpstereo_amd/csrc/les_kernels.h
+++ b/localexpstereo_amd/csrc/les_kernels.h
@@ -245,7 +245,7 @@
 };
 
 #if defined(LES_PHASE_TIMING) && !defined(LES_SIM)
-__device__ unsigned long long les_dbg[12];
+__device__ unsigned long long les_dbg[16];
 #define LES_PHASE_BEGIN() unsigned long long ph_[5] = {0, 0, 0, 0, 0}; unsigned long long tl_ = clock64()
 #define LES_PHASE_MARK(k) do { const unsigned long long now_ = clock64(); ph_[k] += now_ - tl_; tl_ = now_; } while (0)
 #define LES_PHASE_END() do { if (threadIdx.x == 0) { for (int k_ = 0; k_ < 5; k_++) atomicAdd(&les_dbg[k_], ph_[k_]); atomicAdd(&les_dbg[5], 1ull); } } while (0)
diff --git a/localexpstereo_amd/csrc/les_march.h b/localexpstereo_amd/csrc/les_march.h
--- a/localexpstereo_amd/csrc/les_march.h
+++ b/localexpstereo_amd/csrc/les_march.h
@@ -26,6 +26,20 @@
 constexpr int kMarchMagicBits = 0x4B400000;
 static_assert(kMarchSH + kMarchMB + kMarchSL == 32, "N cov = t - hi32(M * (s << SL)) needs the scales to meet at 2^32");
 __host__ __device__ constexpr int march_pb(int R) { return (2 * R + 1) * (2 * R + 1) < 512 ? 20 : 19; }
+
+__host__ __device__ constexpr int march_fdiv(int a, int b) { return a >= 0 ? a / b : -((-a + b - 1) / b); }
+__host__ __device__ constexpr int march_chain_switch(int lag, int BY) { return -march_fdiv(-(lag - BY + 1), BY) - 1; }
+__host__ __device__ constexpr int march_chain_period(int th, int R, int BY)
+{
+    int need = R;
+    for (int lag = 0; lag <= 2 * R; lag += R) {
+        const int gap = lag - march_chain_switch(lag, BY) * BY;
+        need = need > gap ? need : gap;
+    }
+    return (th + need + BY - 1) / BY * BY;
+}
+static_assert(march_chain_period(1000, 10, 7) == 1015 && march_chain_period(41, 10, 7) == 56 && march_chain_period(57, 10, 7) == 70 &&
+              march_chain_period(30, 4, 3) == 36 && march_chain_period(23, 2, 2) == 26, "chain period table of tests/test_march_chain.py");
 #ifndef LES_MARCH_STAT_WORDS
 #define LES_MARCH_STAT_WORDS 9
 #endif
@@ -245,7 +259,7 @@
 template <int R, int WGC, int NJ, int BY>
 __global__ void __launch_bounds__(3 * WGC * NJ)
 les_march_kernel(Geom g, MarchView view, const Job* __restrict__ jobs, const float4* __restrict__ planes,
-                 float* __restrict__ out, int ngroups, int check)
+                 float* __restrict__ out, int ngroups, int check, int chain_len)
 {
     using Cfg = MarchCfg<R, WGC, NJ, BY>;
     constexpr int KS = Cfg::KS, RS = Cfg::RS, NT = Cfg::NT, HWV = Cfg::HWV, PCOLS = Cfg::PCOLS;
@@ -268,12 +282,24 @@
     constexpr int kRoleOf[6][3] = {{0, 1, 2}, {2, 1, 0}, {1, 2, 0}, {2, 0, 1}, {1, 0, 2}, {0, 2, 1}};
     const int slot = wave / (3 * HWV), role = kRoleOf[LES_MARCH_ROLE_ORDER][(wave % (3 * HWV)) / HWV], half = wave % HWV;
     const int ci0 = half * 64, ci = ci0 + lane;
-    const Job job = jobs[grp * NJ + slot];
-    int th_max = 0;
-#pragma unroll
-    for (int s = 0; s < NJ; s++) th_max = max(th_max, jobs[grp * NJ + s].th);
-    const int nblk = (th_max + 4 * R + BY - 1) / BY;
+    const int chain = NJ == 1 ? chain_len : 0;
+    const Job* const cjobs = jobs + (chain ? (long long)grp * chain : (long long)grp * NJ + slot);
+    const Job job = cjobs[0];
+    int nblk;
+    int PB = 0, nchain = 1;
+    if (chain) {
+        nchain = 1;
+        while (nchain < chain && cjobs[nchain].th > 0) nchain++;
+        PB = march_chain_period(job.th, R, BY) / BY;
+        nblk = ((nchain - 1) * PB * BY + job.th + 2 * R + BY - 1) / BY;
+    } else {
+        int th_max = 0;
+#pragma unroll
+        for (int s = 0; s < NJ; s++) th_max = max(th_max, jobs[grp * NJ + s].th);
+        nblk = (th_max + 4 * R + BY - 1) / BY;
+    }
     const int nticks = nblk + 3;
+    const int P = PB * BY;
     const int Ttot = job.th > 0 ? job.th + 4 * R : 0;
     const float4 plane = planes[job.plane_idx];
     const int cy1m = max(job.cy1 - 1, job.cy0);
@@ -285,14 +311,19 @@
     }
     __syncthreads();
 
-    const int gx = job.tx0 - 2 * R + ci;
-    const bool col_in = gx >= job.cx0 && gx < job.cx1 && job.th > 0;
-    const int sx = min(max(gx, job.cx0), max(job.cx1 - 1, job.cx0));
-    const uint32_t sx4 = (uint32_t)sx * 4u;
+    int gx, sx, nx;
+    bool col_in;
+    uint32_t sx4;
+    auto set_cols = [&](const Job& jb) __attribute__((always_inline)) {
+        gx = jb.tx0 - 2 * R + ci;
+        col_in = gx >= jb.cx0 && gx < jb.cx1 && jb.th > 0;
+        sx = min(max(gx, jb.cx0), max(jb.cx1 - 1, jb.cx0));
+        sx4 = (uint32_t)sx * 4u;
+        nx = window_count(gx, R, jb.cx0, jb.cx1);
+    };
     const uint32_t rowB = (uint32_t)g.W * 4u;
     const uint32_t imgB = (uint32_t)g.H * rowB;
     const BufRsrc rs_guide = make_buf(view.ipk8, imgB);
-    const int nx = window_count(gx, R, job.cx0, job.cx1);
     const int cP = min(ci + R, WGC - 1), cM = ci - R - 1;
     const int pcP = Cfg::pcol(cP);
     const int pcM = cM >= 0 ? Cfg::pcol(cM) : 0;
@@ -302,7 +333,6 @@
 
     if (role == 0 && LES_LAB_ROLE_ON(1)) {
         const uint32_t HWu = (uint32_t)g.H * (uint32_t)g.W;
-        const float g_ax = plane.x * (float)sx;
         const bool fronto = plane.x == 0.0f && plane.y == 0.0f;
         GatherPrep gpc = gather_prepare(g, 0.0f, plane.z, 0u, HWu, true);
         if (gpc.f1 == 0.0f) gpc.i1 = gpc.i0;
@@ -317,6 +347,8 @@
         const int modes = readfirstlane_i32(gpc.mode);
         const float f0s = 1.0f - f1s;
         const bool inv_job = fronto && modes == 2 && !view.raw_off;
+        const float sp_in = __int_as_float(readfirstlane_i32(__float_as_int(inv_job ? 0.0f : view.sp)));
+        const float pm_in = __int_as_float(readfirstlane_i32(__float_as_int(inv_job ? fmaf(g.th_col, view.sp, view.pmagic) : view.pmagic)));
         int slice_lo = 0;
         const bool tame = !fronto && !view.raw_off && march_plane_short_gather(g, plane, job, R, &slice_lo);
         const uint32_t W8 = ((uint32_t)g.W + 7u) >> 3;
@@ -326,8 +358,6 @@
         const unsigned long long tspanB = (unsigned long long)max(trow_hi - trow_lo, 1) * (unsigned long long)trowB;
         const bool tiled = tame && view.vol_t && fabsf(plane.x) >= (NJ == 1 ? LES_TILED_MIN_SLOPE_WIDE : LES_TILED_MIN_SLOPE) && tspanB < 0xfffffff0ull &&
                            (unsigned long long)W8 * (unsigned long long)g.D * 32ull < (1ull << 31);
-        const float spj = !col_in ? 0.0f : (inv_job ? 0.0f : view.sp);
-        const float pmj = !col_in ? __int_as_float(kMarchMagicBits) : (inv_job ? fmaf(g.th_col, view.sp, view.pmagic) : view.pmagic);
         auto march_a = [&](auto kind_tag) __attribute__((always_inline)) {
         constexpr int KIND = decltype(kind_tag)::value;
         GatherPrep gp[BY];
@@ -348,11 +378,19 @@
         const unsigned long long trestB = (unsigned long long)(g.H - trow_lo) * (unsigned long long)trowB;
         const uint32_t tiledB = (uint32_t)(trestB < 0xfffffffcull ? trestB : 0xfffffffcull);
         const BufRsrc rs_v0 = make_buf(v0base, KIND == 3 ? 0xfffffffcu : (KIND == 4 ? (uint32_t)(rest4 < 0xfffffffcull ? rest4 : 0xfffffffcull) : (KIND == 5 ? tiledB : imgB)));
-        const uint32_t tcol = (((uint32_t)sx >> 3) * (uint32_t)g.D * 8u + ((uint32_t)sx & 7u)) * 4u;
         const int dsub = g.D0 - slice_lo;
         const BufRsrc rs_v1 = make_buf(view.vol + (size_t)i1s, imgB);
+        LES_TICK_BEGIN();
+        for (int jA = 0; jA < nchain; jA++) {
+        set_cols(cjobs[jA]);
+        const int tsh = chain ? 2 * R - jA * P : 0;
+        const int kbeg = jA == 0 ? 0 : jA * PB - 1, kend = jA + 1 < nchain ? (jA + 1) * PB - 1 : nticks;
+        const float g_ax = plane.x * (float)sx;
+        const float spj = !col_in ? 0.0f : sp_in;
+        const float pmj = !col_in ? __int_as_float(kMarchMagicBits) : pm_in;
+        const uint32_t tcol = (((uint32_t)sx >> 3) * (uint32_t)g.D * 8u + ((uint32_t)sx & 7u)) * 4u;
         auto prep = [&](int b) __attribute__((always_inline)) {
-            const int t = b * BY + lane;
+            const int t = b * BY + lane + tsh;
             const int gy = job.ty0 - 2 * R + t;
             const int sy = min(max(gy, job.cy0), cy1m);
             nx_rowB = (int)((uint32_t)sy * rowB);
@@ -397,16 +435,17 @@
             }
             gw[i] = buf_load<uint32_t>(rs_guide, sx4, ro);
         };
-        prep(0);
-        rowbits = rowbits_nx;
-        prep(0);
-        static_for<BY>([&](auto itag) { issue_row(itag); });
-        LES_TICK_BEGIN();
-        for (int k0 = 0; k0 < nticks; k0 += UN) {
+        if (jA == 0) {
+            prep(0);
+            rowbits = rowbits_nx;
+            prep(0);
+            static_for<BY>([&](auto itag) { issue_row(itag); });
+        }
+        for (int k0 = kbeg - kbeg % UN; k0 < kend; k0 += UN) {
             static_for<UN>([&](auto utag) {
                 constexpr int BASE = decltype(utag)::value * BY;
                 const int k = k0 + decltype(utag)::value;
-                if (k < nticks) {
+                if (k >= kbeg && k < kend) {
                     if (k < nblk) {
                         int4 (*T)[PCOLS] = s_T1[k & 1][slot];
                         prep(k + 1);
@@ -461,6 +500,7 @@
                 }
             });
         }
+        }
         LES_TICK_END(0);
         };
         if (view.raw_off) march_a(std::integral_constant<int, 3>{});
@@ -470,12 +510,19 @@
         else if (tame) march_a(std::integral_constant<int, 4>{});
         else march_a(std::integral_constant<int, 2>{});
     } else if (role == 1 && LES_LAB_ROLE_ON(2)) {
-        const bool s1_col = col_in && ci >= R && ci < WGC - R;
         int slice_lo_unused = 0;
         const bool general_plane = !view.raw_off && !(plane.x == 0.0f && plane.y == 0.0f) && !march_plane_short_gather(g, plane, job, R, &slice_lo_unused);
-        const float kap_x = s1_col ? view.kapS * s_rtab[nx] : 0.0f;
-        const float up_x = s1_col ? view.upS * s_rtab[nx] : 0.0f;
-        const uint32_t sxS = (uint32_t)sx * (uint32_t)(4 * kMarchStatWords);
+        float kap_x, up_x;
+        uint32_t sxS;
+        auto set_cols_c = [&]() __attribute__((always_inline)) {
+            const bool s1_col = col_in && ci >= R && ci < WGC - R;
+            kap_x = s1_col ? view.kapS * s_rtab[nx] : 0.0f;
+            up_x = s1_col ? view.upS * s_rtab[nx] : 0.0f;
+            sxS = (uint32_t)sx * (uint32_t)(4 * kMarchStatWords);
+        };
+        set_cols(job);
+        set_cols_c();
+        int tsh = chain ? 2 * R : 0, jC = 0, swC = nchain > 1 ? PB + march_chain_switch(R, BY) : -1;
         const uint32_t rowS = (uint32_t)g.W * (uint32_t)(4 * kMarchStatWords);
         const MarchStatDesc ds_stats = march_stats_desc(view.mstats, (uint32_t)g.H * rowS);
         MarchStatRow st[BY];
@@ -492,7 +539,7 @@
         int nx_srow = 0;
         float nx_rny = 0.0f;
         auto prep = [&](int b) __attribute__((always_inline)) {
-            const int t = b * BY + lane;
+            const int t = b * BY + lane + tsh;
             const int gy1 = job.ty0 - 3 * R + t;
             const bool on = gy1 >= job.cy0 && gy1 < job.cy1 && t >= 2 * R && t < Ttot;
             nx_rny = on ? s_rtab[window_count(gy1, R, job.cy0, job.cy1)] : 0.0f;
@@ -512,6 +559,13 @@
         for (int k = 0; k < nticks; k++) {
             if (k >= 1 && k <= nblk) {
                 const int b = k - 1;
+                if (b == swC) {
+                    jC++;
+                    tsh -= P;
+                    swC = jC + 1 < nchain ? swC + PB : -1;
+                    set_cols(cjobs[jC]);
+                    set_cols_c();
+                }
                 const int4 (*T1)[PCOLS] = s_T1[b & 1][slot];
                 int4 (*T2)[PCOLS] = s_T2[b % 3][slot];
                 constexpr int GC = 2, NS = (BY + GC - 1) / GC;
@@ -568,10 +622,20 @@
         }
         LES_TICK_END(1);
     } else if (role == 2 && LES_LAB_ROLE_ON(4)) {
-        const bool out_col = ci >= 2 * R && ci < 2 * R + job.tw && job.th > 0;
+        bool out_col;
+        float vl_xa, c_lane;
+        BufRsrc rs_out;
         const uint32_t oc4 = (uint32_t)max(ci - 2 * R, 0) * 4u;
-        const float vl_xa = (float)gx * plane.x, vl_c = 1.0f * plane.z, vl_zv = 0.0f * plane.w, vl_a5 = plane.x * 5, vl_b5 = plane.y * 5;
-        const float c_lane = view.qscale * s_rtab[nx];
+        const float vl_c = 1.0f * plane.z, vl_zv = 0.0f * plane.w, vl_a5 = plane.x * 5, vl_b5 = plane.y * 5;
+        auto set_cols_d = [&](const Job& jb) __attribute__((always_inline)) {
+            out_col = ci >= 2 * R && ci < 2 * R + jb.tw && jb.th > 0;
+            vl_xa = (float)gx * plane.x;
+            c_lane = view.qscale * s_rtab[nx];
+            rs_out = make_buf(out + jb.out_off, 0xfffffffcu);
+        };
+        set_cols(job);
+        set_cols_d(job);
+        int tsh = chain ? 2 * R : 0, jD = 0, swD = nchain > 1 ? PB + march_chain_switch(2 * R, BY) : -1;
         int ring2[4][RS];
 #pragma unroll
         for (int k = 0; k < RS; k++) ring2[0][k] = ring2[1][k] = ring2[2][k] = ring2[3][k] = 0;
@@ -581,10 +645,9 @@
         uint32_t okbits = 0;
         int nx_grow = 0;
         float nx_rny = 0.0f;
-        const BufRsrc rs_out = make_buf(out + job.out_off, 0xfffffffcu);
         const uint32_t ostrideB = (uint32_t)job.out_stride * 4u;
         auto prep = [&](int b) __attribute__((always_inline)) {
-            const int t = b * BY + lane;
+            const int t = b * BY + lane + tsh;
             const int gy2 = job.ty0 - 4 * R + t;
             nx_rny = s_rtab[window_count(gy2, R, job.cy0, job.cy1)];
             nx_grow = (int)((uint32_t)min(max(gy2, job.cy0), cy1m) * rowB);
@@ -607,6 +670,14 @@
                 if (k < nticks) {
                     if (k >= 3) {
                         const int b = k - 3;
+                        if (b == swD) {
+                            jD++;
+                            tsh -= P;
+                            swD = jD + 1 < nchain ? swD + PB : -1;
+                            const Job jb = cjobs[jD];
+                            set_cols(jb);
+                            set_cols_d(jb);
+                        }
                         const int4 (*T2)[PCOLS] = s_T2[(U + UN - 3 % UN) % UN][slot];
                         constexpr int GD = 1, NS = (BY + GD - 1) / GD;
                         int4 pp[2][GD], pm[2][GD], px[2][GD];
@@ -636,7 +707,7 @@
                                 ring2[0][SLOT] = h0; ring2[1][SLOT] = h1; ring2[2][SLOT] = h2; ring2[3][SLOT] = h3;
                                 acc64_add_i32(S2[0], h0 - o0); acc64_add_i32(S2[1], h1 - o1); acc64_add_i32(S2[2], h2 - o2); acc64_add_i32(S2[3], h3 - o3);
                                 if (out_col && ((okbits >> i) & 1u)) {
-                                    const int t = b * BY + i;
+                                    const int t = b * BY + i + tsh;
                                     const uint32_t gi = gq[i];
                                     const float f0 = (float)(int)(S2[0] >> kMarchS2), f1 = (float)(int)(S2[1] >> kMarchS2), f2 = (float)(int)(S2[2] >> kMarchS2), f3 = (float)(int)(S2[3] >> kMarchS2);
                                     const float acc = fmaf(f2, cvt_f32_sbyte<2>(gi), fmaf(f1, cvt_f32_sbyte<1>(gi), fmaf(f0, cvt_f32_sbyte<0>(gi), f3 * 255.0f)));
@@ -666,7 +737,11 @@
         }
         LES_TICK_END(2);
         };
-        const bool surely_valid = march_label_surely_valid(g, plane, job.tx0, job.tx0 + max(job.tw, 1) - 1, job.ty0, job.ty0 + max(job.th, 1) - 1);
+        bool surely_valid = true;
+        for (int j = 0; j < nchain; j++) {
+            const Job jb = cjobs[j];
+            surely_valid = surely_valid && march_label_surely_valid(g, plane, jb.tx0, jb.tx0 + max(jb.tw, 1) - 1, jb.ty0, jb.ty0 + max(jb.th, 1) - 1);
+        }
         if (check && !surely_valid) march_d(std::integral_constant<int, 1>{});
         else march_d(std::integral_constant<int, 0>{});
     }
diff --git a/localexpstereo_amd/csrc/les_march_lab.h b/localexpstereo_amd/csrc/les_march_lab.h
--- a/localexpstereo_amd/csrc/les_march_lab.h
+++ b/localexpstereo_amd/csrc/les_march_lab.h
@@ -17,8 +17,10 @@
 #define LES_LAB_ABLATE(bit) ((LES_MARCH_EXP & (bit)) != 0)
 
 #if defined(LES_PHASE_TIMING) && !defined(LES_SIM)
-#define LES_TICK_BEGIN() unsigned long long tk_c_ = 0, tk_w_ = 0, tk_n_ = 0, tk_r_ = 0, tk_m_ = 0, tk_t_ = clock64()
+#define LES_TICK_BEGIN() unsigned long long tk_c_ = 0, tk_w_ = 0, tk_n_ = 0, tk_r_ = 0, tk_m_ = 0, tk_f_ = 0, tk_l_ = 0, tk_a_ = 0, tk_t_ = clock64()
 #define LES_TICK_MARK() (tk_m_ = clock64())
-#define LES_TICK_BARRIER() do { const unsigned long long a_ = clock64(); __syncthreads(); const unsigned long long b_ = clock64(); tk_c_ += a_ - tk_t_; tk_r_ += (tk_m_ > tk_t_ ? tk_m_ : a_) - tk_t_; tk_w_ += b_ - a_; tk_t_ = b_; tk_n_++; } while (0)
-#define LES_TICK_END(role_) do { if (lane == 0) { atomicAdd(&les_dbg[2 * (role_)], tk_c_); atomicAdd(&les_dbg[2 * (role_) + 1], tk_w_); atomicAdd(&les_dbg[6 + (role_)], tk_n_); atomicAdd(&les_dbg[9 + (role_)], tk_r_); } } while (0)
+#define LES_TICK_BARRIER() do { const unsigned long long a_ = clock64(); __syncthreads(); const unsigned long long b_ = clock64(); tk_c_ += a_ - tk_t_; tk_r_ += (tk_m_ > tk_t_ ? tk_m_ : a_) - tk_t_; tk_w_ += b_ - a_; \
+    if (tk_n_ < 9ull) tk_f_ += b_ - tk_t_; if (tk_n_ + 9ull >= (unsigned long long)nticks) tk_l_ += b_ - tk_t_; tk_a_ += b_ - tk_t_; tk_t_ = b_; tk_n_++; } while (0)
+#define LES_TICK_END(role_) do { if (lane == 0) { atomicAdd(&les_dbg[2 * (role_)], tk_c_); atomicAdd(&les_dbg[2 * (role_) + 1], tk_w_); atomicAdd(&les_dbg[6 + (role_)], tk_n_); atomicAdd(&les_dbg[9 + (role_)], tk_r_); \
+    if ((role_) == 0) { atomicAdd(&les_dbg[12], tk_f_); atomicAdd(&les_dbg[13], tk_l_); atomicAdd(&les_dbg[14], tk_a_); atomicAdd(&les_dbg[15], tk_n_); } } } while (0)
 #endif
```

After: 172,500, median of 6. 1.03x the previous value.
